# guanjq/targetdiff

Measured on NVIDIA H100. Metric: molecules/sec (1000-step sampling, CrossDocked pocket shape), higher is better.
Workload: dtype f32 (storage, LayerNorm, softmax, accumulation); GEMM operands as 2-piece bf16 splits on wgmma (3 products, ~16-bit operand mantissa)

## Files before the change

### targetdiff_b200/csrc/edge_mlp_v4.cu

```cuda
#include <stdio.h>
#include <stdlib.h>
#include <string.h>

#include "tdiff_common.cuh"
#include "hopper_mma.cuh"

namespace v4 {

constexpr int kCons = 2;
constexpr int kThreads = (kCons + 1) * 128;
constexpr int kTile = 64;
constexpr int kTabClassBytes = 2 * 128 * 128;
constexpr int kProdRegs = 40, kConsRegs = 232;
constexpr int kSrcStride = 512 + 32, kDst = 8;
constexpr int sSrc = 0, sDstRows = sSrc + kTile * kSrcStride, sMeta = sDstRows + kDst * 512, kStage = sMeta + kTile * 16;
constexpr int kMAtom = 32 * 128, kMPiece = 2 * kMAtom, kMImg = 2 * kMPiece;
template <bool FOLD>
struct Map {
  static constexpr int W = 0, T = W + 4 * 128 * 128, Par = T + (FOLD ? 1 : 2) * kTabClassBytes, X = Par + 2 * 128 * 4,
                       M = X + kCons * 4 * 2 * 128 * 4, C = M + (FOLD ? kCons * kMImg : 0), Stage = C + (FOLD ? kCons * 32 * 4 : 0),
                       Bar = Stage + kCons * kStage, Smem = Bar + 8 * (1 + 2 * kCons);
  static_assert(M % 1024 == 0 && Stage % 128 == 0 && kStage % 128 == 0 && Smem <= 227 * 1024, "shared-memory map");
};
constexpr int kOrderBar = 5;
constexpr int kFoldBar = 7;

__device__ __forceinline__ uint32_t smem_u32(const void* p) { return (uint32_t)__cvta_generic_to_shared(p); }
__device__ __forceinline__ void mbar_init(uint32_t bar, uint32_t count) {
  asm volatile("mbarrier.init.shared::cta.b64 [%0], %1;" ::"r"(bar), "r"(count) : "memory");
}
__device__ __forceinline__ void mbar_wait(uint32_t bar, uint32_t parity) {
  asm volatile(
      "{\n\t.reg .pred p;\n\tWAIT_LOOP:\n\tmbarrier.try_wait.parity.shared::cta.b64 p, [%0], %1;\n\t@p bra WAIT_DONE;\n\tbra WAIT_LOOP;\n\t"
      "WAIT_DONE:\n\t}" ::"r"(bar), "r"(parity) : "memory");
}
__device__ __forceinline__ void mbar_expect_tx(uint32_t bar, uint32_t bytes) {
  asm volatile("mbarrier.arrive.expect_tx.shared::cta.b64 _, [%0], %1;" ::"r"(bar), "r"(bytes) : "memory");
}
__device__ __forceinline__ void bulk_g2s(uint32_t smem_dst, const void* gsrc, uint32_t bytes, uint32_t bar) {
  asm volatile("cp.async.bulk.shared::cluster.global.mbarrier::complete_tx::bytes [%0], [%1], %2, [%3];" ::"r"(smem_dst), "l"(gsrc), "r"(bytes),
               "r"(bar) : "memory");
}
__device__ __forceinline__ void fence_barrier_init() { asm volatile("fence.mbarrier_init.release.cluster;" ::: "memory"); }
__device__ __forceinline__ void mbar_arrive(uint32_t bar) { asm volatile("mbarrier.arrive.shared::cta.b64 _, [%0];" ::"r"(bar) : "memory"); }
__device__ __forceinline__ void mbar_expect_tx_only(uint32_t bar, uint32_t bytes) {
  asm volatile("mbarrier.expect_tx.shared::cta.b64 [%0], %1;" ::"r"(bar), "r"(bytes) : "memory");
}
__device__ __forceinline__ void named_bar_sync(int id, int nthreads) { asm volatile("bar.sync %0, %1;" ::"r"(id), "r"(nthreads) : "memory"); }
__device__ __forceinline__ void named_bar_arrive(int id, int nthreads) { asm volatile("bar.arrive %0, %1;" ::"r"(id), "r"(nthreads) : "memory"); }
template <int N> __device__ __forceinline__ void setmaxnreg_inc() { asm volatile("setmaxnreg.inc.sync.aligned.u32 %0;" ::"n"(N)); }
template <int N> __device__ __forceinline__ void setmaxnreg_dec() { asm volatile("setmaxnreg.dec.sync.aligned.u32 %0;" ::"n"(N)); }

__device__ __forceinline__ uint32_t cvt_bf16x2(float hi, float lo) {
  uint32_t d;
  asm("cvt.rn.bf16x2.f32 %0, %1, %2;" : "=r"(d) : "f"(hi), "f"(lo));
  return d;
}
__device__ __forceinline__ float ex2_approx(float x) { float y; asm("ex2.approx.ftz.f32 %0, %1;" : "=f"(y) : "f"(x)); return y; }
__device__ __forceinline__ void stg64(float* p, float a, float b) { asm volatile("st.global.v2.f32 [%0], {%1,%2};" ::"l"(p), "f"(a), "f"(b) : "memory"); }
__device__ __forceinline__ void stg128(float* p, float a, float b, float c, float d) {
  asm volatile("st.global.v4.f32 [%0], {%1,%2,%3,%4};" ::"l"(p), "f"(a), "f"(b), "f"(c), "f"(d) : "memory");
}

struct LnParams { float b[128]; float b2[128]; float mu[20]; };
struct AggArgs {
  const float* logits;
  const float* e_w;
  float* h;
  int key_softmax;
};

template <int N, int M, int LO_BIT>
__device__ __forceinline__ void transpose_reduce(float (&t)[N], int lane) {
  if constexpr (N > M) {
    constexpr int h = (N / M / 2) << LO_BIT;
    const bool up = lane & h;
#pragma unroll
    for (int i = 0; i < N / 2; ++i) {
      const float send = up ? t[i] : t[i + N / 2];
      const float keep = up ? t[i + N / 2] : t[i];
      t[i] = keep + __shfl_xor_sync(0xffffffffu, send, h);
    }
    transpose_reduce<N / 2, M, LO_BIT>(reinterpret_cast<float(&)[N / 2]>(t), lane);
  }
}
__device__ __forceinline__ void split2(float y0, float y1, uint32_t& hi, uint32_t& lo) {
  hi = cvt_bf16x2(y1, y0);
  const float r0 = __fsub_rn(y0, __uint_as_float(hi << 16)), r1 = __fsub_rn(y1, __uint_as_float(hi & 0xffff0000u));
  lo = cvt_bf16x2(r1, r0);
}

}

using namespace v4;

template <int NOUT, bool FOLD>
__global__ void __launch_bounds__(kThreads, 1)
edge_mlp_v4_kernel(const float* __restrict__ P, int zero_row, const int* __restrict__ src, const unsigned char* __restrict__ etype,
                   const float* __restrict__ dist_arr, const int* __restrict__ row_nodes, long long n_dst, long long split_dst,
                   const int* __restrict__ d_counts, int k, int offA, int offB, const unsigned char* __restrict__ w2_image,
                   const unsigned char* __restrict__ tab_image, float coeff, const float* __restrict__ qnode, float* __restrict__ out, int out_by_slot, AggArgs agg,
                   int fold_cls, const __grid_constant__ LnParams lp) {
  static_assert(!FOLD || NOUT == 128, "the fold applies to the key MLPs");
  using L = Map<FOLD>;
  extern __shared__ __align__(1024) unsigned char smem_raw[];
  const uint32_t sbase = smem_u32(smem_raw);
  const uint32_t sW = sbase + L::W, sT = sbase + L::T, sBar = sbase + L::Bar;
  float* const s_b = reinterpret_cast<float*>(smem_raw + L::Par);
  float* const s_b2 = s_b + 128;
  const int tid = threadIdx.x, lane = tid & 31, warp = __shfl_sync(0xffffffffu, tid >> 5, 0);
  const int w = warp & 3, q = lane & 3;
  const int kshift = (k & (k - 1)) == 0 ? __ffs(k) - 1 : -1;
  auto row_dst = [&](long long idx, int& j) -> unsigned {
    const unsigned a = kshift >= 0 ? (unsigned)idx >> kshift : (unsigned)idx / (unsigned)k;
    j = (int)((unsigned)idx - a * (unsigned)k);
    return a;
  };

  if ((sbase & 1023u) != 0) __trap();
  if (d_counts) { n_dst = d_counts[0]; split_dst = d_counts[1]; }
  const long long n_rows = n_dst * k, split_rows = split_dst * k;
  long long row_lo = 0, row_hi = n_rows;
  if constexpr (FOLD) { if (fold_cls) row_lo = split_rows; else row_hi = split_rows; }
  const long long n_tiles = row_hi > row_lo ? (row_hi - row_lo + kTile - 1) / kTile : 0;
  const long long my_tiles = (n_tiles > blockIdx.x) ? (n_tiles - blockIdx.x + gridDim.x - 1) / gridDim.x : 0;
  auto full_bar = [&](int c) { return sBar + 8u * (1 + c); };
  auto empty_bar = [&](int c) { return sBar + 8u * (1 + kCons + c); };

  constexpr int kWAtom = NOUT * 128;
  constexpr int kWPiece = 2 * kWAtom;
  if (tid == 0) {
    mbar_init(sBar, 1);
    for (int c = 0; c < kCons; ++c) { mbar_init(full_bar(c), 32); mbar_init(empty_bar(c), 128); }
    fence_barrier_init();
    if constexpr (FOLD) {
      mbar_expect_tx(sBar, 4u * 128 * 128 + kTabClassBytes);
      bulk_g2s(sW, w2_image, 4u * 128 * 128, sBar);
      bulk_g2s(sT, tab_image + (size_t)fold_cls * kTabClassBytes, kTabClassBytes, sBar);
    } else {
      mbar_expect_tx(sBar, 2u * kWPiece + 2u * kTabClassBytes);
      bulk_g2s(sW, w2_image, 2u * kWPiece, sBar);
      bulk_g2s(sT, tab_image, 2u * kTabClassBytes, sBar);
    }
  }
  for (int i = tid; i < 128; i += kThreads) { s_b[i] = lp.b[i]; s_b2[i] = lp.b2[i]; }
  __syncthreads();

  if (warp < 4) {
    setmaxnreg_dec<kProdRegs>();
    if (warp >= kCons) return;
    const int c = warp;
    const uint32_t st = sbase + L::Stage + (uint32_t)c * kStage;
    for (long long it = c, use = 0; it < my_tiles; it += kCons, ++use) {
      const long long tile = blockIdx.x + it * (long long)gridDim.x, row0 = row_lo + tile * kTile;
      int j0;
      const unsigned a0 = row_dst(row0, j0);
      const long long last = (row0 + kTile - 1 < row_hi ? row0 + kTile - 1 : row_hi - 1);
      const int n_d = min(kDst, (int)(row_dst(last, j0) - a0) + 1);
      int s[2];
      int4 meta[2];
#pragma unroll
      for (int h = 0; h < 2; ++h) {
        const long long idx = row0 + lane + 32 * h;
        int jj = 0, ty = 3, slot = 0, node = -1;
        float dist = 0.f;
        s[h] = -1;
        if (idx < n_rows) {
          const unsigned a = row_dst(idx, jj);
          slot = a - a0 < (unsigned)kDst ? (int)(a - a0) + 1 : 0;
          node = row_nodes[a];
          if (node >= 0) {
            const size_t e = (size_t)node * k + jj;
            s[h] = src[e]; ty = etype[e]; dist = dist_arr[e];
          }
        }
        meta[h] = make_int4(node, s[h], __float_as_int(dist), ty | (slot << 8) | (jj << 16));
      }
      int dnode = -1;
      if (lane < n_d) dnode = row_nodes[a0 + lane];
      mbar_wait(empty_bar(c), (uint32_t)(use & 1) ^ 1u);
#pragma unroll
      for (int h = 0; h < 2; ++h) *reinterpret_cast<int4*>(smem_raw + L::Stage + c * kStage + sMeta + 16 * (lane + 32 * h)) = meta[h];
      if (lane == 0) mbar_expect_tx_only(full_bar(c), (uint32_t)(kTile + (FOLD ? 2 : 1) * n_d) * 512u);
      __syncwarp();
#pragma unroll
      for (int h = 0; h < 2; ++h)
        bulk_g2s(st + sSrc + (uint32_t)(lane + 32 * h) * kSrcStride, P + (size_t)(s[h] >= 0 ? s[h] : zero_row) * TD_NPROJ + offB, 512u, full_bar(c));
      if (lane < n_d) bulk_g2s(st + sDstRows + (uint32_t)lane * 512u, P + (size_t)(dnode >= 0 ? dnode : zero_row) * TD_NPROJ + offA, 512u, full_bar(c));
      if (FOLD && lane < n_d) bulk_g2s(st + sDstRows + (uint32_t)(2 + lane) * 512u, qnode + (size_t)(dnode >= 0 ? dnode : 0) * TD_H, 512u, full_bar(c));
      mbar_arrive(full_bar(c));
    }
    return;
  }

  setmaxnreg_inc<kConsRegs>();
  const int cwg = (warp >> 2) - 1;
  float mu[5];
#pragma unroll
  for (int m = 0; m < 5; ++m) mu[m] = lp.mu[5 * q + m];
  const float coeff2 = coeff * 1.4426950408889634f;
  mbar_wait(sBar, 0);

  const int r_base = 16 * w + (lane >> 2);
  const int pair_bar = 1 + 2 * cwg + (w >> 1);
  float* const xslot = reinterpret_cast<float*>(smem_raw + L::X) + (size_t)(cwg * 4 + w) * 256;
  float* const xpart = xslot + ((w & 1) ? -256 : 256);
  const bool do_agg = !FOLD && NOUT == 128 && qnode == nullptr && agg.logits != nullptr;
  const bool key_sm = NOUT == 128 && qnode != nullptr && agg.key_softmax;
  const unsigned char* const stage = smem_raw + L::Stage + cwg * kStage;
  const int ct = tid & 127, fu = ct & 7, fg = ct >> 3;
  const int fhd = 8 * (fg & 1) + 4 * (fu >> 2) + (fu & 3), fs = fu >> 2, frun = (fg >> 1) ^ (((fu >> 1) & 1) << 2);
  const int fn0 = 16 * ((fhd >> 1) & 1) + 2 * (fhd >> 2) + (fhd & 1);
  unsigned char* const mimg = smem_raw + L::M + cwg * kMImg;
  float* const s_c = reinterpret_cast<float*>(smem_raw + L::C) + cwg * 32;
  const int srow = k == 32 ? (w >> 1) : 0;
  const int order_mine = kOrderBar + cwg, order_other = kOrderBar + (cwg ^ 1);
  const long long n_iter = (my_tiles + kCons - 1) / kCons;
  if (n_iter == 0) return;
  if (cwg == 1) named_bar_arrive(order_other, 256);
  int set = 0;

  for (long long n = 0; n < n_iter; ++n, set ^= 1) {
    const long long it = n * kCons + cwg;
    if (it >= my_tiles) {
      for (int phase = 0; phase < 2; ++phase) { named_bar_sync(order_mine, 256); named_bar_arrive(order_other, 256); }
      continue;
    }
    const long long tile = blockIdx.x + it * (long long)gridDim.x, row0 = row_lo + tile * kTile;
    const int cls = FOLD ? 0 : (row0 >= split_rows) ? 1 : 0;
    long long idx[2];
    int node[2], s[2], ty[2], jj[2], dsl[2];
    float dist[2];
    mbar_wait(full_bar(cwg), (uint32_t)(n & 1));
#pragma unroll
    for (int h = 0; h < 2; ++h) {
      idx[h] = row0 + r_base + 8 * h;
      const int4 m4 = *reinterpret_cast<const int4*>(stage + sMeta + 16 * (r_base + 8 * h));
      node[h] = m4.x; s[h] = m4.y; dist[h] = __int_as_float(m4.z);
      ty[h] = m4.w & 0xff; dsl[h] = ((m4.w >> 8) & 0xff) - 1; jj[h] = m4.w >> 16;
    }
    float ewp[2] = {0.f, 0.f};
    float4 qf[2][2];
    if constexpr (FOLD) {
#pragma unroll
      for (int h = 0; h < 2; ++h)
        if (key_sm && idx[h] < n_rows && node[h] >= 0) ewp[h] = agg.e_w[(size_t)node[h] * k + jj[h]];
#pragma unroll
      for (int sl = 0; sl < 2; ++sl)
#pragma unroll
        for (int hf = 0; hf < 2; ++hf) {
          float4 v = make_float4(0.f, 0.f, 0.f, 0.f);
          if (sl == 0 || k == 32) {
            v = *reinterpret_cast<const float4*>(stage + sDstRows + (2 + sl) * 512 + 32 * fhd + 16 * (hf ^ fs));
            v.x *= 0.35355339059327373f; v.y *= 0.35355339059327373f; v.z *= 0.35355339059327373f; v.w *= 0.35355339059327373f;
          }
          qf[sl][hf] = v;
        }
    }
    uint32_t ghi[4][4], glo[4][4];
#pragma unroll
    for (int h = 0; h < 2; ++h) {
      const bool ok = s[h] >= 0;
      float v[8];
#pragma unroll
      for (int m = 0; m < 5; ++m) {
        const float t = dist[h] - mu[m];
        v[m] = ok ? ex2_approx(coeff2 * (t * t)) : 0.0f;
      }
      v[5] = (ok && q == 3) ? 1.0f : 0.0f;
      v[6] = v[7] = 0.0f;
      const int half = ty[h] < 2 ? 1 : 0;
#pragma unroll
      for (int kk = 0; kk < 4; ++kk)
#pragma unroll
        for (int hk = 0; hk < 2; ++hk) {
          uint32_t hi, lo;
          split2(v[4 * (kk & 1) + 2 * hk], v[4 * (kk & 1) + 2 * hk + 1], hi, lo);
          const bool own = (kk >> 1) == half;
          ghi[kk][h + 2 * hk] = own ? hi : 0u;
          glo[kk][h + 2 * hk] = own ? lo : 0u;
        }
    }
    float x[64];
#pragma unroll
    for (int h = 0; h < 2; ++h) {
      const bool valid = s[h] >= 0;
      const float* ps = reinterpret_cast<const float*>(stage + sSrc + (r_base + 8 * h) * kSrcStride) + 2 * q;
      const float* pd = (dsl[h] >= 0 ? reinterpret_cast<const float*>(stage + sDstRows + dsl[h] * 512)
                                     : P + (size_t)(valid ? node[h] : zero_row) * TD_NPROJ + offA) + 2 * q;
#pragma unroll
      for (int i = 0; i < 16; ++i) {
        const float2 b = *reinterpret_cast<const float2*>(ps + 8 * i);
        float2 a = make_float2(0.f, 0.f);
        if (valid) a = *reinterpret_cast<const float2*>(pd + 8 * i);
        x[4 * i + 2 * h] = __fadd_rn(b.x, a.x);
        x[4 * i + 2 * h + 1] = __fadd_rn(b.y, a.y);
      }
    }
    mbar_arrive(empty_bar(cwg));
    const uint32_t sTc = sT + (uint32_t)cls * kTabClassBytes;
    wgmma_fence();
    named_bar_sync(order_mine, 256);
#pragma unroll
    for (int term = 0; term < 3; ++term) {
#pragma unroll
      for (int kk = 0; kk < 4; ++kk)
        wgmma_n128_rs(x, term == 2 ? glo[kk] : ghi[kk], gmma_desc_sw128(sTc + (term == 1 ? kTabClassBytes / 2 : 0) + kk * 32),
                      1u);
    }
    wgmma_commit();
    named_bar_arrive(order_other, 256);
    if constexpr (FOLD) {
      const float* const w2s = reinterpret_cast<const float*>(smem_raw + L::W) + 8 * fhd;
#pragma unroll
      for (int jr = 0; jr < 2; ++jr) {
        const int f0 = 64 * jr + 8 * frun;
        float mv[2][8];
#pragma unroll
        for (int jf = 0; jf < 8; ++jf) {
          const float4 wa = *reinterpret_cast<const float4*>(w2s + (f0 + jf) * 128 + 4 * fs);
          const float4 wb = *reinterpret_cast<const float4*>(w2s + (f0 + jf) * 128 + 4 * (fs ^ 1));
#pragma unroll
          for (int sl = 0; sl < 2; ++sl) {
            const float4 qa = qf[sl][0], qb = qf[sl][1];
            const float pa = __fmaf_rn(wa.w, qa.w, __fmaf_rn(wa.z, qa.z, __fmaf_rn(wa.y, qa.y, wa.x * qa.x)));
            const float pb = __fmaf_rn(wb.w, qb.w, __fmaf_rn(wb.z, qb.z, __fmaf_rn(wb.y, qb.y, wb.x * qb.x)));
            mv[sl][jf] = pa + pb;
          }
        }
#pragma unroll
        for (int sl = 0; sl < 2; ++sl) {
          uint4 hi, lo;
          split2(mv[sl][0], mv[sl][1], hi.x, lo.x);
          split2(mv[sl][2], mv[sl][3], hi.y, lo.y);
          split2(mv[sl][4], mv[sl][5], hi.z, lo.z);
          split2(mv[sl][6], mv[sl][7], hi.w, lo.w);
          const int nr = fn0 + 8 * sl;
          const int off = jr * kMAtom + (nr >> 3) * 1024 + (nr & 7) * 128 + ((frun ^ (nr & 7)) << 4);
          *reinterpret_cast<uint4*>(mimg + off) = hi;
          *reinterpret_cast<uint4*>(mimg + kMPiece + off) = lo;
        }
      }
      if (fg < 2)
#pragma unroll
        for (int sl = 0; sl < 2; ++sl) {
          const float4 ba = *reinterpret_cast<const float4*>(s_b2 + 8 * fhd + 4 * fs), bb = *reinterpret_cast<const float4*>(s_b2 + 8 * fhd + 4 * (fs ^ 1));
          const float4 qa = qf[sl][0], qb = qf[sl][1];
          const float pa = __fmaf_rn(ba.w, qa.w, __fmaf_rn(ba.z, qa.z, __fmaf_rn(ba.y, qa.y, ba.x * qa.x)));
          const float pb = __fmaf_rn(bb.w, qb.w, __fmaf_rn(bb.z, qb.z, __fmaf_rn(bb.y, qb.y, bb.x * qb.x)));
          s_c[16 * sl + fhd] = pa + pb;
        }
      asm volatile("fence.proxy.async.shared::cta;" ::: "memory");
    }
    wgmma_wait_all();
    float rstd[2];
#pragma unroll
    for (int h = 0; h < 2; ++h) {
      float qa = 0.f, qb = 0.f;
#pragma unroll
      for (int i = 0; i < 16; ++i) {
        qa = __fmaf_rn(x[4 * i + 2 * h], x[4 * i + 2 * h], qa);
        qb = __fmaf_rn(x[4 * i + 2 * h + 1], x[4 * i + 2 * h + 1], qb);
      }
      float var = qa + qb;
      var += __shfl_xor_sync(0xffffffffu, var, 1);
      var += __shfl_xor_sync(0xffffffffu, var, 2);
      rstd[h] = rsqrtf(var * (1.0f / 128.0f) + 1e-5f);
    }
    uint32_t ahi[8][4], alo[8][4];
#pragma unroll
    for (int kk = 0; kk < 8; ++kk)
#pragma unroll
      for (int r = 0; r < 4; ++r) {
        const int h = r & 1, col = 16 * kk + 8 * (r >> 1) + 2 * q, e = 8 * kk + 2 * r;
        const float2 b = *reinterpret_cast<const float2*>(s_b + col);
        const float y0 = __fmaf_rn(x[e], rstd[h], b.x), y1 = __fmaf_rn(x[e + 1], rstd[h], b.y);
        split2(fmaxf(y0, 0.f), fmaxf(y1, 0.f), ahi[kk][r], alo[kk][r]);
      }
    float o[NOUT / 2];
    if constexpr (FOLD) {
      named_bar_sync(kFoldBar + cwg, 128);
#pragma unroll
      for (int sl = 0; sl < 2; ++sl) {
        const float4 cv = *reinterpret_cast<const float4*>(s_c + 16 * sl + 4 * q);
#pragma unroll
        for (int h = 0; h < 2; ++h) {
          o[4 * sl + 2 * h] = cv.x; o[4 * sl + 2 * h + 1] = cv.y;
          o[4 * (2 + sl) + 2 * h] = cv.z; o[4 * (2 + sl) + 2 * h + 1] = cv.w;
        }
      }
    }
    wgmma_fence();
    named_bar_sync(order_mine, 256);
#pragma unroll
    for (int term = 0; term < 3; ++term) {
#pragma unroll
      for (int kk = 0; kk < 8; ++kk) {
        if constexpr (FOLD) {
          const uint64_t desc = gmma_desc_sw128(sbase + L::M + cwg * kMImg + (term == 1 ? kMPiece : 0) + (kk >> 2) * kMAtom + (kk & 3) * 32);
          wgmma_n32_rs(reinterpret_cast<float(&)[16]>(o), term == 2 ? alo[kk] : ahi[kk], desc, 1u);
        } else {
          const uint64_t desc = gmma_desc_sw128(sW + (term == 1 ? kWPiece : 0) + (kk >> 2) * kWAtom + (kk & 3) * 32);
          if constexpr (NOUT == 128) wgmma_n128_rs(o, term == 2 ? alo[kk] : ahi[kk], desc, (term | kk) ? 1u : 0u);
          else wgmma_n16_rs(o, term == 2 ? alo[kk] : ahi[kk], desc, (term | kk) ? 1u : 0u);
        }
      }
    }
    wgmma_commit();
    named_bar_arrive(order_other, 256);
    wgmma_wait_all();

    long long orow[2];
    bool owrite[2];
#pragma unroll
    for (int h = 0; h < 2; ++h) {
      orow[h] = out_by_slot ? ((long long)node[h] * k + jj[h]) : idx[h];
      owrite[h] = idx[h] < n_rows && node[h] >= 0;
    }
    if constexpr (NOUT == 16) {
#pragma unroll
      for (int h = 0; h < 2; ++h)
        if (owrite[h])
#pragma unroll
          for (int i = 0; i < 2; ++i) {
            const float2 bb = *reinterpret_cast<const float2*>(s_b2 + 8 * i + 2 * q);
            stg64(out + (size_t)orow[h] * 16 + 8 * i + 2 * q, o[4 * i + 2 * h] + bb.x, o[4 * i + 2 * h + 1] + bb.y);
          }
    } else if (do_agg) {
      const long long dslot = tile * 2 + (w >> 1);
      const int dnode = dslot < n_dst ? row_nodes[dslot] : -1;
      const bool active = dnode >= 0;
      const int ccol = 64 * (w & 1) + 2 * lane;
      float2 hin = make_float2(0.f, 0.f);
      if (active) hin = *reinterpret_cast<const float2*>(agg.h + (size_t)dnode * TD_H + ccol);
      float wt[2][16];
#pragma unroll
      for (int h = 0; h < 2; ++h)
#pragma unroll
        for (int i = 0; i < 4; ++i) {
          float4 t4 = make_float4(0.f, 0.f, 0.f, 0.f);
          if (active) t4 = __ldg(reinterpret_cast<const float4*>(agg.logits + (size_t)idx[h] * TD_HEADS + 4 * i));
          wt[h][4 * i] = t4.x; wt[h][4 * i + 1] = t4.y; wt[h][4 * i + 2] = t4.z; wt[h][4 * i + 3] = t4.w;
        }
      float t[32];
#pragma unroll
      for (int i = 0; i < 16; ++i) {
        const float2 bb = *reinterpret_cast<const float2*>(s_b2 + 8 * i + 2 * q);
#pragma unroll
        for (int c = 0; c < 2; ++c) {
          const float b = c ? bb.y : bb.x;
          t[2 * i + c] = __fadd_rn(__fmul_rn(__fadd_rn(o[4 * i + c], b), wt[0][i]), __fmul_rn(__fadd_rn(o[4 * i + 2 + c], b), wt[1][i]));
        }
      }
      transpose_reduce<32, 4, 2>(t, lane);
      float* slot = xslot + 128 * set;
      const int c0 = 16 * (lane >> 2) + 2 * q;
      *reinterpret_cast<float2*>(slot + c0) = make_float2(t[0], t[1]);
      *reinterpret_cast<float2*>(slot + c0 + 8) = make_float2(t[2], t[3]);
      named_bar_sync(pair_bar, 64);
      if (active) {
        const float* se = ((w & 1) ? xpart : xslot) + 128 * set;
        const float* so = ((w & 1) ? xslot : xpart) + 128 * set;
        const float2 a = *reinterpret_cast<const float2*>(se + ccol), b = *reinterpret_cast<const float2*>(so + ccol);
        *reinterpret_cast<float2*>(agg.h + (size_t)dnode * TD_H + ccol) = make_float2(hin.x + (a.x + b.x), hin.y + (a.y + b.y));
      }
    } else if (!FOLD && qnode == nullptr) {
#pragma unroll
      for (int h = 0; h < 2; ++h)
        if (owrite[h])
#pragma unroll
          for (int i = 0; i < 16; ++i) {
            const float2 bb = *reinterpret_cast<const float2*>(s_b2 + 8 * i + 2 * q);
            stg64(out + (size_t)orow[h] * 128 + 8 * i + 2 * q, o[4 * i + 2 * h] + bb.x, o[4 * i + 2 * h + 1] + bb.y);
          }
    } else {
      float lg[32];
      if constexpr (FOLD) {
#pragma unroll
        for (int h = 0; h < 2; ++h)
#pragma unroll
          for (int u = 0; u < 4; ++u) {
            const int e0 = 4 * (2 * (u >> 1)) + 2 * h + (u & 1);
            lg[4 * h + u] = srow ? o[e0 + 4] : o[e0];
          }
      } else {
#pragma unroll
        for (int h = 0; h < 2; ++h) {
          const float* qrow = qnode + (size_t)(node[h] >= 0 ? node[h] : 0) * TD_H + 2 * q;
#pragma unroll
          for (int i = 0; i < 16; ++i) {
            const float2 qv = __ldg(reinterpret_cast<const float2*>(qrow + 8 * i));
            const float2 bb = *reinterpret_cast<const float2*>(s_b2 + 8 * i + 2 * q);
            lg[8 * (i >> 2) + 4 * h + (i & 3)] = __fmaf_rn(o[4 * i + 2 * h + 1] + bb.y, qv.y, (o[4 * i + 2 * h] + bb.x) * qv.x);
          }
        }
        transpose_reduce<32, 8, 0>(lg, lane);
#pragma unroll
        for (int u = 0; u < 8; ++u) lg[u] *= 0.35355339059327373f;
      }
      if (key_sm) {
        bool valid_e[2];
        float ew[2];
#pragma unroll
        for (int h = 0; h < 2; ++h) {
          valid_e[h] = false; ew[h] = 0.f;
          if (owrite[h]) {
            valid_e[h] = s[h] >= 0;
            ew[h] = FOLD ? ewp[h] : agg.e_w[(size_t)node[h] * k + jj[h]];
          }
        }
        float mx[4], sm[4];
#pragma unroll
        for (int u = 0; u < 4; ++u) {
          lg[u] = valid_e[0] ? lg[u] * 1.4426950408889634f : -INFINITY;
          lg[4 + u] = valid_e[1] ? lg[4 + u] * 1.4426950408889634f : -INFINITY;
          mx[u] = fmaxf(lg[u], lg[4 + u]);
#pragma unroll
          for (int m = 4; m < 32; m <<= 1) mx[u] = fmaxf(mx[u], __shfl_xor_sync(0xffffffffu, mx[u], m));
        }
        if (lane < 4) *reinterpret_cast<float4*>(xslot + 4 * q) = make_float4(mx[0], mx[1], mx[2], mx[3]);
        named_bar_sync(pair_bar, 64);
        const float4 pm = *reinterpret_cast<const float4*>(xpart + 4 * q);
        mx[0] = fmaxf(mx[0], pm.x); mx[1] = fmaxf(mx[1], pm.y); mx[2] = fmaxf(mx[2], pm.z); mx[3] = fmaxf(mx[3], pm.w);
#pragma unroll
        for (int u = 0; u < 4; ++u) {
          lg[u] = valid_e[0] ? ex2_approx(lg[u] - mx[u]) : 0.0f;
          lg[4 + u] = valid_e[1] ? ex2_approx(lg[4 + u] - mx[u]) : 0.0f;
          sm[u] = lg[u] + lg[4 + u];
#pragma unroll
          for (int m = 4; m < 32; m <<= 1) sm[u] += __shfl_xor_sync(0xffffffffu, sm[u], m);
        }
        if (lane < 4) *reinterpret_cast<float4*>(xslot + 128 + 4 * q) = make_float4(sm[0], sm[1], sm[2], sm[3]);
        named_bar_sync(pair_bar, 64);
        const float4 ps = *reinterpret_cast<const float4*>(xpart + 128 + 4 * q);
        const float pl[4] = {ps.x, ps.y, ps.z, ps.w};
#pragma unroll
        for (int u = 0; u < 4; ++u) {
          const float l = sm[u] + pl[u];
          const float inv = l > 0.0f ? 1.0f / l : 0.0f;
          lg[u] = lg[u] * ew[0] * inv;
          lg[4 + u] = lg[4 + u] * ew[1] * inv;
        }
#pragma unroll
        for (int h = 0; h < 2; ++h)
          if (idx[h] < n_rows) stg128(out + (size_t)idx[h] * TD_HEADS + 4 * q, lg[4 * h], lg[4 * h + 1], lg[4 * h + 2], lg[4 * h + 3]);
      } else {
#pragma unroll
        for (int h = 0; h < 2; ++h)
          if (owrite[h]) stg128(out + (size_t)orow[h] * TD_HEADS + 4 * q, lg[4 * h], lg[4 * h + 1], lg[4 * h + 2], lg[4 * h + 3]);
      }
    }
  }
  if (cwg == 0) named_bar_sync(order_mine, 256);
}

void td_launch_edge_mlp_v4(const float* P, int zero_row, const int* src, const unsigned char* etype, const float* dist, const int* row_nodes, long long n_dst,
                           long long split_dst, const int* d_counts, int k, const TdMlp& m, const float* h_offsets, float coeff,
                           const float* h_ln_b, const float* h_b2, const float* qnode, float* out, int out_by_slot,
                           const float* agg_logits, const float* agg_e_w, float* agg_h, int key_softmax, int sm_count, cudaStream_t st) {
  if (n_dst == 0) return;
  LnParams lp;
  memcpy(lp.b, h_ln_b, sizeof(lp.b));
  memset(lp.b2, 0, sizeof(lp.b2));
  memcpy(lp.b2, h_b2, sizeof(float) * (size_t)m.nout);
  memcpy(lp.mu, h_offsets, sizeof(lp.mu));
  static size_t opted128[TD_MAX_DEVICES] = {0}, opted16[TD_MAX_DEVICES] = {0}, optedF[TD_MAX_DEVICES] = {0};
  td_opt_in_smem(edge_mlp_v4_kernel<128, false>, Map<false>::Smem, opted128);
  td_opt_in_smem(edge_mlp_v4_kernel<16, false>, Map<false>::Smem, opted16);
  td_opt_in_smem(edge_mlp_v4_kernel<128, true>, Map<true>::Smem, optedF);
  auto grid_of = [&](long long n_dst_range) {
    const long long n_tiles = (n_dst_range * k + kTile - 1) / kTile;
    return (int)(n_tiles < sm_count ? n_tiles : sm_count);
  };
  AggArgs agg = {agg_logits, agg_e_w, agg_h, (key_softmax && k == 32) ? 1 : 0};
  if (m.nout == 16) {
    edge_mlp_v4_kernel<16, false><<<grid_of(n_dst), kThreads, Map<false>::Smem, st>>>(
        P, zero_row, src, etype, dist, row_nodes, n_dst, split_dst, d_counts, k, m.offA, m.offB, m.w2_img, m.tabcls_img, coeff, nullptr, out,
        out_by_slot, agg, 0, lp);
  } else if (qnode && (k == 32 || k == 64)) {
    const long long n_cls[2] = {split_dst, n_dst - split_dst};
    for (int cls = 0; cls < 2; ++cls)
      if (n_cls[cls] > 0)
        edge_mlp_v4_kernel<128, true><<<grid_of(n_cls[cls]), kThreads, Map<true>::Smem, st>>>(
            P, zero_row, src, etype, dist, row_nodes, n_dst, split_dst, d_counts, k, m.offA, m.offB,
            reinterpret_cast<const unsigned char*>(m.w2t), m.tabcls_img, coeff, qnode, out, out_by_slot, agg, cls, lp);
  } else {
    edge_mlp_v4_kernel<128, false><<<grid_of(n_dst), kThreads, Map<false>::Smem, st>>>(
        P, zero_row, src, etype, dist, row_nodes, n_dst, split_dst, d_counts, k, m.offA, m.offB, m.w2_img, m.tabcls_img, coeff, qnode, out,
        out_by_slot, agg, 0, lp);
  }
}
```

### targetdiff_b200/csrc/engine.cu

```cuda
#include <math.h>
#include <stdarg.h>
#include <stdio.h>
#include <stdlib.h>
#include <string.h>

#include <list>
#include <map>
#include <string>
#include <vector>

#include "../../include/tdiff.h"
#include "sampler.cuh"
#include "tdiff_common.cuh"

static thread_local char g_err[1024] = "";
static int set_err(int code, const char* fmt, ...) {
  va_list ap;
  va_start(ap, fmt);
  vsnprintf(g_err, sizeof(g_err), fmt, ap);
  va_end(ap);
  return code;
}
#define CK(call)                                                                                       \
  do {                                                                                                 \
    cudaError_t _e = (call);                                                                           \
    if (_e != cudaSuccess) return set_err(TDIFF_ECUDA, "%s failed: %s (%s:%d)", #call, cudaGetErrorString(_e), __FILE__, __LINE__); \
  } while (0)

struct DevBuf {
  void* p = nullptr;
  size_t cap = 0;
  int ensure(size_t bytes) {
    if (bytes <= cap) return 0;
    if (p) cudaFree(p);
    p = nullptr; cap = 0;
    size_t want = bytes + bytes / 8 + 256;
    if (cudaMalloc(&p, want) != cudaSuccess) { (void)cudaGetLastError(); if (cudaMalloc(&p, bytes) != cudaSuccess) { (void)cudaGetLastError(); return -1; } want = bytes; }
    cap = want;
    static const bool poison = getenv("TDIFF_POISON") != nullptr;
    if (poison) cudaMemset(p, 0xFF, want);
    return 0;
  }
  void release() { if (p) cudaFree(p); p = nullptr; cap = 0; }
  template <class T> T* as() const { return reinterpret_cast<T*>(p); }
};

struct TdLayer {
  std::vector<TdSubLayer> x2h, h2x;
  const float* offsets;
  float coeff;
};

enum { EV_AGG_H = 0, EV_AGG_X = 1, EV_EDGE_MLP = 2, EV_TOTAL = 3, EV_KINDS = 4 };
struct EvPair { cudaEvent_t a, b; int kind; };

struct tdiff_engine {
  tdiff_config cfg;
  int device = 0, sm_count = 132;
  float* arena = nullptr;
  std::vector<float> host_arena;
  unsigned char* img_arena = nullptr;
  int mlp_mode = 2;
  bool mlp_v4 = true;
  std::vector<TdLayer> layers;
  const float *w_prot = nullptr, *b_prot = nullptr, *wl_t = nullptr, *bl = nullptr;
  const float *ew_w1t = nullptr, *ew_b1 = nullptr, *ew_g = nullptr, *ew_b = nullptr, *ew_w2 = nullptr, *ew_off = nullptr;
  float ew_b2 = 0.f, ew_coeff = -0.5f;
  int num_blocks = 1, ew_mode = 0 , out_fc = 0, time_emb = 0;
  int num_x2h = 1, num_h2x = 1, sync_twoup = 0;
  const float* w_time = nullptr;
  const float* zeros128 = nullptr;
  DevBuf ew_x2h, ew_h2x, hagg, time_norm;
  DevBuf h_sync;
  const float *hd_w1t = nullptr, *hd_b1 = nullptr, *hd_w2 = nullptr, *hd_b2 = nullptr;
  const float *t_c0 = nullptr, *t_ct = nullptr, *t_logvar = nullptr, *t_la = nullptr, *t_l1ma = nullptr, *t_lca = nullptr, *t_l1mca = nullptr,
              *t_sra = nullptr, *t_srm1 = nullptr;
  bool bound = false, has_ligand = false, have_graph = false;
  bool restrict_last = false;
  bool knn_incremental = false;
  bool have_prev = false;
  bool env_no_fused_agg = false, env_no_restrict = false, env_no_graph = false, env_knn_full = false, env_no_slot_keep = false;
  int B = 0, N = 0, Np = 0, Nl = 0, K = 0, max_ng = 0, final_buf = 0;
  int KQ = 0, hybrid = 0;
  DevBuf node_ptr, prot_ptr, prot_node, prot_graph, lig_node, lig_graph, node_lig;
  DevBuf rel_flag, rel_list, n_rel, work_list, n_work, knn_cache;
  DevBuf x2h_rows, lig_rows, rel_rows, rel_counts;
  long long x2h_n_dst = 0, x2h_split = 0, lig_n_dst = 0;
  int row_pad = 4;
  int free_depth = 0;
  int env_free_depth = 2;
  bool free_ready = false;
  DevBuf h_free, dirty, free_rows, free_counts, lig_save;
  long long free_stride = 0;
  DevBuf xm0, xm1, offset, h0, h, P, q, src, src_prev, etype, e_w, dist, kbuf, vbuf, v16, lig_pos, lig_v, logits;
  DevBuf step, err_flag, node_off, total_edges;
  DevBuf stage[8];
  cudaStream_t own_stream = nullptr;
  cudaEvent_t ev_fork = nullptr, ev_join = nullptr;
  long long launches = 0;
  bool profiling = false;
  std::vector<EvPair> events;
  double ms_acc[EV_KINDS] = {0, 0, 0, 0};
  long long n_acc[EV_KINDS] = {0, 0, 0, 0};
};

namespace {
struct Packer {
  std::map<std::string, const tdiff_tensor*> byname;
  std::vector<float> host;
  std::vector<unsigned char> img;
  std::string missing;
  std::list<std::vector<float>> keep;
  const float* get(const std::string& name, int64_t numel) {
    auto it = byname.find(name);
    if (it == byname.end() || it->second->numel != numel || it->second->data == nullptr) {
      if (missing.empty()) missing = name + (it == byname.end() ? " (absent)" : " (wrong size)");
      return nullptr;
    }
    return it->second->data;
  }
  size_t alloc(size_t n) {
    size_t off = (host.size() + 63) / 64 * 64;
    host.resize(off + n, 0.0f);
    return off;
  }
};

struct MlpOff { size_t tab, ln_g, ln_b, w2t, b2; int nout; long long img, tabcls; };

inline uint16_t bf16_rn(float x) {
  uint32_t u; memcpy(&u, &x, 4);
  if ((u & 0x7fffffffu) > 0x7f800000u) return (uint16_t)((u >> 16) | 0x40);
  u += 0x7fffu + ((u >> 16) & 1u);
  return (uint16_t)(u >> 16);
}
inline float bf16_f(uint16_t b) { uint32_t u = (uint32_t)b << 16; float f; memcpy(&f, &u, 4); return f; }

void pack_umma_image(const float* w2, std::vector<unsigned char>& img, size_t off, int nrows = 128) {
  for (int n = 0; n < nrows; ++n)
    for (int kk = 0; kk < 128; ++kk) {
      float r = w2[(size_t)n * 128 + kk];
      const size_t o = (size_t)(kk / 64) * ((size_t)nrows * 128) + (size_t)n * 128 + (size_t)((((kk % 64) / 8) ^ (n & 7)) * 16) + (size_t)(kk % 8) * 2;
      for (int p = 0; p < 3; ++p) {
        const uint16_t b = bf16_rn(r);
        r = r - bf16_f(b);
        memcpy(&img[off + (size_t)p * ((size_t)nrows * 256) + o], &b, 2);
      }
    }
}

void pack_tabcls_image(const float* tab , std::vector<unsigned char>& img, size_t off) {
  static const int type_of[2][2] = {{3, 1}, {2, 0}};
  for (int cls = 0; cls < 2; ++cls)
    for (int n = 0; n < 128; ++n)
      for (int slot = 0; slot < 64; ++slot) {
        const int half = slot >> 5, sl = slot & 31;
        const int q = (sl & 7) >> 1, m = 2 * (sl >> 3) + (sl & 1);
        int j = -1;
        if (m < 5) j = 5 * q + m;
        else if (m == 5 && q == 3) j = 20;
        float r = j >= 0 ? tab[((size_t)type_of[cls][half] * TD_TAB + j) * TD_H + n] : 0.0f;
        const size_t o = (size_t)n * 128 + (size_t)(((slot >> 3) ^ (n & 7)) * 16) + (size_t)(slot & 7) * 2;
        for (int p = 0; p < 2; ++p) {
          const uint16_t b = bf16_rn(r);
          r = r - bf16_f(b);
          memcpy(&img[off + (size_t)cls * 32768 + (size_t)p * 16384 + o], &b, 2);
        }
      }
}

bool pack_edge_mlp(Packer& pk, const std::string& p, int nout, bool sign_in_w1, MlpOff& o, const float** w1_out) {
  const int KV = 4 + 4 * TD_NG + 2 * TD_H;
  const float* w1_in = pk.get(p + ".net.0.weight", (int64_t)TD_H * KV);
  const float* b1_in = pk.get(p + ".net.0.bias", TD_H);
  const float* g_in = pk.get(p + ".net.1.weight", TD_H);
  const float* b_in = pk.get(p + ".net.1.bias", TD_H);
  const float* w2_in = pk.get(p + ".net.3.weight", (int64_t)nout * TD_H);
  const float* b2_in = pk.get(p + ".net.3.bias", nout);
  if (!w1_in || !b1_in || !g_in || !b_in || !w2_in || !b2_in) return false;
  std::vector<float>& w1v = pk.keep.emplace_back((size_t)TD_H * KV);
  std::vector<float> b1v(TD_H), gv(TD_H), bv(TD_H), w2v((size_t)nout * TD_H), b2v(nout);
  {
    std::vector<double> mw(KV, 0.0), b2acc(b2_in, b2_in + nout);
    double mb = 0.0;
    for (int f = 0; f < TD_H; ++f) {
      for (int j = 0; j < KV; ++j) mw[j] += w1_in[(size_t)f * KV + j];
      mb += b1_in[f];
    }
    for (int f = 0; f < TD_H; ++f) {
      const double s = g_in[f] < 0.0f ? -1.0 : 1.0, ag = fabs((double)g_in[f]), s1 = sign_in_w1 ? s : 1.0;
      for (int j = 0; j < KV; ++j) w1v[(size_t)f * KV + j] = (float)(s1 * (w1_in[(size_t)f * KV + j] - mw[j] / TD_H));
      b1v[f] = (float)(s1 * (b1_in[f] - mb / TD_H));
      gv[f] = (float)(s / s1);
      const float bf = (float)(b_in[f] / ag);
      const bool constant = g_in[f] == 0.0f || !isfinite(bf);
      bv[f] = constant ? 0.0f : bf;
      for (int n = 0; n < nout; ++n) {
        const double w = w2_in[(size_t)n * TD_H + f];
        w2v[(size_t)n * TD_H + f] = constant ? 0.0f : (float)(ag * w);
        if (constant && b_in[f] > 0.0f) b2acc[n] += (double)b_in[f] * w;
      }
    }
    for (int n = 0; n < nout; ++n) b2v[n] = (float)b2acc[n];
  }
  const float *w1 = w1v.data(), *b1 = b1v.data(), *g = gv.data(), *b = bv.data(), *w2 = w2v.data(), *b2 = b2v.data();
  o.nout = nout;
  o.tab = pk.alloc(4 * TD_TAB * TD_H);
  for (int t = 0; t < 4; ++t) {
    for (int j = 0; j < TD_NG; ++j)
      for (int f = 0; f < TD_H; ++f) pk.host[o.tab + (t * TD_TAB + j) * TD_H + f] = w1[(size_t)f * KV + 4 + t * TD_NG + j];
    for (int f = 0; f < TD_H; ++f) pk.host[o.tab + (t * TD_TAB + TD_NG) * TD_H + f] = w1[(size_t)f * KV + t] + b1[f];
  }
  o.ln_g = pk.alloc(TD_H); memcpy(&pk.host[o.ln_g], g, TD_H * sizeof(float));
  o.ln_b = pk.alloc(TD_H); memcpy(&pk.host[o.ln_b], b, TD_H * sizeof(float));
  o.w2t = pk.alloc((size_t)TD_H * nout);
  for (int kk = 0; kk < TD_H; ++kk)
    for (int n = 0; n < nout; ++n) pk.host[o.w2t + (size_t)kk * nout + n] = w2[(size_t)n * TD_H + kk];
  o.b2 = pk.alloc(nout); memcpy(&pk.host[o.b2], b2, nout * sizeof(float));
  o.img = -1; o.tabcls = -1;
  if (nout == TD_H || nout == 16) {
    o.img = (long long)pk.img.size();
    pk.img.resize(pk.img.size() + 3 * (size_t)nout * 256, 0);
    pack_umma_image(w2, pk.img, (size_t)o.img, nout);
    o.tabcls = (long long)pk.img.size();
    pk.img.resize(pk.img.size() + 2 * 32768, 0);
    pack_tabcls_image(&pk.host[o.tab], pk.img, (size_t)o.tabcls);
  }
  *w1_out = w1;
  return true;
}

struct SubOff {
  size_t wn_t, bn; long long wn_img; MlpOff k, v, q;
  long long ew_w = -1; float ew_b = 0.f;
  long long out_wa = -1, out_wb = -1, out_w2 = -1, out_b1 = -1, out_g = -1, out_b = -1, out_b2 = -1;
};

bool pack_sublayer_options(Packer& pk, const std::string& p, int ew_dim, bool out_fc, SubOff& so) {
  if (ew_dim > 0) {
    const float* w = pk.get(p + ".ew_net.0.weight", ew_dim);
    const float* b = pk.get(p + ".ew_net.0.bias", 1);
    if (!w || !b) return false;
    so.ew_w = (long long)pk.alloc(ew_dim);
    memcpy(&pk.host[so.ew_w], w, ew_dim * sizeof(float));
    so.ew_b = b[0];
  }
  if (out_fc) {
    const std::string np = p + ".node_output";
    const float* w1 = pk.get(np + ".net.0.weight", (int64_t)TD_H * 2 * TD_H);
    const float* b1 = pk.get(np + ".net.0.bias", TD_H);
    const float* g = pk.get(np + ".net.1.weight", TD_H);
    const float* b = pk.get(np + ".net.1.bias", TD_H);
    const float* w2 = pk.get(np + ".net.3.weight", (int64_t)TD_H * TD_H);
    const float* b2 = pk.get(np + ".net.3.bias", TD_H);
    if (!w1 || !b1 || !g || !b || !w2 || !b2) return false;
    std::vector<float> blk((size_t)TD_H * TD_H);
    for (int half = 0; half < 2; ++half) {
      for (int n = 0; n < TD_H; ++n)
        for (int kk = 0; kk < TD_H; ++kk) blk[(size_t)n * TD_H + kk] = w1[(size_t)n * 2 * TD_H + half * TD_H + kk];
      long long& dst = half == 0 ? so.out_wa : so.out_wb;
      dst = (long long)pk.img.size();
      pk.img.resize(pk.img.size() + 3 * 32768, 0);
      pack_umma_image(blk.data(), pk.img, (size_t)dst);
    }
    so.out_w2 = (long long)pk.img.size();
    pk.img.resize(pk.img.size() + 3 * 32768, 0);
    pack_umma_image(w2, pk.img, (size_t)so.out_w2);
    so.out_b1 = (long long)pk.alloc(TD_H); memcpy(&pk.host[so.out_b1], b1, TD_H * 4);
    so.out_g = (long long)pk.alloc(TD_H); memcpy(&pk.host[so.out_g], g, TD_H * 4);
    so.out_b = (long long)pk.alloc(TD_H); memcpy(&pk.host[so.out_b], b, TD_H * 4);
    so.out_b2 = (long long)pk.alloc(TD_H); memcpy(&pk.host[so.out_b2], b2, TD_H * 4);
  }
  return true;
}

bool pack_sublayer(Packer& pk, const std::string& p, const char* kn, const char* vn, const char* qn, int nout_v, bool sign_in_w1, SubOff& so) {
  const int KV = 4 + 4 * TD_NG + 2 * TD_H;
  const float *w1k = nullptr, *w1v = nullptr;
  if (!pack_edge_mlp(pk, p + "." + kn, TD_H, sign_in_w1, so.k, &w1k)) return false;
  if (!pack_edge_mlp(pk, p + "." + vn, nout_v, sign_in_w1, so.v, &w1v)) return false;
  const std::string qp = p + "." + qn;
  const float* w1q = pk.get(qp + ".net.0.weight", (int64_t)TD_H * TD_H);
  const float* b1q = pk.get(qp + ".net.0.bias", TD_H);
  const float* gq = pk.get(qp + ".net.1.weight", TD_H);
  const float* bq = pk.get(qp + ".net.1.bias", TD_H);
  const float* w2q = pk.get(qp + ".net.3.weight", (int64_t)TD_H * TD_H);
  const float* b2q = pk.get(qp + ".net.3.bias", TD_H);
  if (!w1q || !b1q || !gq || !bq || !w2q || !b2q) return false;
  so.q.nout = TD_H; so.q.tab = 0; so.q.tabcls = -1;
  so.q.img = (long long)pk.img.size();
  pk.img.resize(pk.img.size() + 3 * 32768, 0);
  pack_umma_image(w2q, pk.img, (size_t)so.q.img);
  so.q.ln_g = pk.alloc(TD_H); memcpy(&pk.host[so.q.ln_g], gq, TD_H * sizeof(float));
  so.q.ln_b = pk.alloc(TD_H); memcpy(&pk.host[so.q.ln_b], bq, TD_H * sizeof(float));
  so.q.w2t = pk.alloc((size_t)TD_H * TD_H);
  for (int kk = 0; kk < TD_H; ++kk)
    for (int n = 0; n < TD_H; ++n) pk.host[so.q.w2t + (size_t)kk * TD_H + n] = w2q[(size_t)n * TD_H + kk];
  so.q.b2 = pk.alloc(TD_H); memcpy(&pk.host[so.q.b2], b2q, TD_H * sizeof(float));
  so.wn_t = pk.alloc((size_t)TD_H * TD_NPROJ);
  so.bn = pk.alloc(TD_NPROJ);
  for (int kk = 0; kk < TD_H; ++kk) {
    float* row = &pk.host[so.wn_t + (size_t)kk * TD_NPROJ];
    for (int c = 0; c < TD_H; ++c) {
      row[c] = w1k[(size_t)c * KV + 4 + 4 * TD_NG + kk];
      row[128 + c] = w1v[(size_t)c * KV + 4 + 4 * TD_NG + kk];
      row[256 + c] = w1k[(size_t)c * KV + 4 + 4 * TD_NG + TD_H + kk];
      row[384 + c] = w1v[(size_t)c * KV + 4 + 4 * TD_NG + TD_H + kk];
      row[512 + c] = w1q[(size_t)c * TD_H + kk];
    }
  }
  for (int c = 0; c < TD_H; ++c) pk.host[so.bn + 512 + c] = b1q[c];
  so.wn_img = (long long)pk.img.size();
  pk.img.resize(pk.img.size() + 5 * 3 * 32768, 0);
  std::vector<float> blk((size_t)TD_H * TD_H);
  for (int y = 0; y < 5; ++y) {
    for (int n = 0; n < TD_H; ++n)
      for (int kk = 0; kk < TD_H; ++kk) blk[(size_t)n * TD_H + kk] = pk.host[so.wn_t + (size_t)kk * TD_NPROJ + y * TD_H + n];
    pack_umma_image(blk.data(), pk.img, (size_t)so.wn_img + (size_t)y * 3 * 32768);
  }
  return true;
}

TdMlp mk_mlp(const float* base, const unsigned char* img_base, const MlpOff& o, int offA, int offB) {
  TdMlp m;
  m.w2_img = (o.img >= 0 && img_base) ? img_base + o.img : nullptr;
  m.tabcls_img = (o.tabcls >= 0 && img_base) ? img_base + o.tabcls : nullptr;
  m.tab = base + o.tab; m.ln_g = base + o.ln_g; m.ln_b = base + o.ln_b; m.w2t = base + o.w2t; m.b2 = base + o.b2;
  m.nout = o.nout; m.offA = offA; m.offB = offB;
  return m;
}
}

extern "C" const char* tdiff_last_error(void) { return g_err; }
extern "C" const char* tdiff_version(void) { return "tdiff-b200 0.1 (sm_90a)"; }

extern "C" int tdiff_create(const tdiff_config* cfg, const tdiff_tensor* sd, int n_entries, int device, tdiff_engine** out) {
  if (!cfg || !sd || !out) return set_err(TDIFF_EINVAL, "null argument");
  *out = nullptr;
  if (cfg->hidden_dim != TD_H || cfg->n_heads != TD_HEADS || cfg->num_r_gaussian != TD_NG)
    return set_err(TDIFF_EINVAL, "unsupported model shape: hidden_dim=%d n_heads=%d num_r_gaussian=%d (kernels are built for 128/16/20)",
                   cfg->hidden_dim, cfg->n_heads, cfg->num_r_gaussian);
  if (cfg->knn < 1 || cfg->knn > TD_KMAX) return set_err(TDIFF_EINVAL, "knn=%d outside 1..%d", cfg->knn, TD_KMAX);
  if (cfg->model_mean_type != 0 && cfg->model_mean_type != 1)
    return set_err(TDIFF_EINVAL, "model_mean_type=%d (0 = C0, 1 = noise)", cfg->model_mean_type);
  for (int r : cfg->reserved)
    if (r != 0) return set_err(TDIFF_EINVAL, "tdiff_config.reserved must be 0");
  int num_x2h = 1, num_h2x = 1, sync_twoup = 0;
  if (cfg->sublayers != 0) {
    const unsigned s = (unsigned)cfg->sublayers;
    num_x2h = (int)(s & 0xffu); num_h2x = (int)((s >> 8) & 0xffu); sync_twoup = (int)((s >> 16) & 0xffu);
    if ((s >> 24) != 1u || num_x2h > 16 || num_h2x > 16 || sync_twoup > 1)
      return set_err(TDIFF_EINVAL, "sublayers=0x%08x: expected 0 or 1<<24 | sync_twoup<<16 | num_h2x<<8 | num_x2h with num_x2h, num_h2x in 0..16 and "
                     "sync_twoup in 0..1", s);
  }
  if (cfg->cutoff_mode != 0 && cfg->cutoff_mode != 1) return set_err(TDIFF_EINVAL, "cutoff_mode=%d (0 = 'knn', 1 = 'hybrid')", cfg->cutoff_mode);
  if (cfg->num_blocks < 0 || cfg->num_blocks > 16 || cfg->ew_net_type < 0 || cfg->ew_net_type > 3 || (cfg->x2h_out_fc != 0 && cfg->x2h_out_fc != 1) ||
      (cfg->time_emb != 0 && cfg->time_emb != 1))
    return set_err(TDIFF_EINVAL, "bad option (num_blocks=%d ew_net_type=%d x2h_out_fc=%d time_emb=%d)", cfg->num_blocks, cfg->ew_net_type,
                   cfg->x2h_out_fc, cfg->time_emb);
  if (cfg->num_layers < 1 || cfg->num_classes < 1 || cfg->num_classes > TD_CMAX || cfg->protein_feat_dim < 1 || cfg->num_timesteps < 1)
    return set_err(TDIFF_EINVAL, "bad config (num_layers=%d num_classes=%d protein_feat_dim=%d num_timesteps=%d)", cfg->num_layers,
                   cfg->num_classes, cfg->protein_feat_dim, cfg->num_timesteps);
  int ndev = 0;
  if (cudaGetDeviceCount(&ndev) != cudaSuccess || ndev == 0) {
    (void)cudaGetLastError();
    return set_err(TDIFF_ECUDA, "no CUDA device: libtdiff has no CPU fallback");
  }
  if (device < 0 || device >= ndev) return set_err(TDIFF_EINVAL, "device %d out of range (%d devices)", device, ndev);
  CK(cudaSetDevice(device));
  cudaDeviceProp prop;
  CK(cudaGetDeviceProperties(&prop, device));
  if (prop.major != 9) return set_err(TDIFF_ECUDA, "device %d is sm_%d%d; this library is built for sm_90a only", device, prop.major, prop.minor);

  tdiff_engine* e = new tdiff_engine();
  e->cfg = *cfg; e->device = device; e->sm_count = prop.multiProcessorCount; e->K = e->KQ = cfg->knn; e->hybrid = cfg->cutoff_mode;
  e->num_blocks = cfg->num_blocks > 1 ? cfg->num_blocks : 1; e->ew_mode = cfg->ew_net_type; e->out_fc = cfg->x2h_out_fc; e->time_emb = cfg->time_emb;
  e->num_x2h = num_x2h; e->num_h2x = num_h2x; e->sync_twoup = sync_twoup;
  if (const char* mode = getenv("TDIFF_EDGE_MLP")) {
    if (!strcmp(mode, "simt")) e->mlp_mode = 0;
    else if (!strcmp(mode, "tc3")) e->mlp_mode = 2;
    else if (!strcmp(mode, "tc3v2")) { e->mlp_mode = 2; e->mlp_v4 = false; }
    else if (!strcmp(mode, "tc6")) e->mlp_mode = 3;
    else { delete e; return set_err(TDIFF_EINVAL, "TDIFF_EDGE_MLP=%s (simt|tc3|tc3v2|tc6)", mode); }
  }
  const bool v4 = e->mlp_mode == 2 && e->mlp_v4;

  Packer pk;
  for (int i = 0; i < n_entries; ++i)
    if (sd[i].name) pk.byname[sd[i].name] = &sd[i];
  const int T = cfg->num_timesteps, KC = cfg->num_classes, F = cfg->protein_feat_dim, L = cfg->num_layers;
  struct { const char* name; size_t off; } tabs[9] = {{"posterior_mean_c0_coef", 0}, {"posterior_mean_ct_coef", 0}, {"posterior_logvar", 0},
      {"log_alphas_v", 0}, {"log_one_minus_alphas_v", 0}, {"log_alphas_cumprod_v", 0}, {"log_one_minus_alphas_cumprod_v", 0},
      {"sqrt_recip_alphas_cumprod", 0}, {"sqrt_recipm1_alphas_cumprod", 0}};
  for (auto& t : tabs) {
    const float* p = pk.get(t.name, T);
    t.off = pk.alloc(T);
    if (p) memcpy(&pk.host[t.off], p, T * sizeof(float));
  }
  const float* wp = pk.get("protein_atom_emb.weight", (int64_t)(TD_H - 1) * F);
  const float* bp = pk.get("protein_atom_emb.bias", TD_H - 1);
  const int KIN = KC + (cfg->time_emb ? 1 : 0);
  const float* wl = pk.get("ligand_atom_emb.weight", (int64_t)(TD_H - 1) * KIN);
  const float* blp = pk.get("ligand_atom_emb.bias", TD_H - 1);
  size_t o_wp = pk.alloc((size_t)TD_H * F), o_bp = pk.alloc(TD_H), o_wl = pk.alloc((size_t)KC * TD_H), o_bl = pk.alloc(TD_H),
         o_wtime = pk.alloc(TD_H), o_zeros = pk.alloc(TD_H);
  if (wp && bp && wl && blp) {
    memcpy(&pk.host[o_wp], wp, (size_t)(TD_H - 1) * F * sizeof(float));
    memcpy(&pk.host[o_bp], bp, (TD_H - 1) * sizeof(float));
    for (int v = 0; v < KC; ++v)
      for (int f = 0; f < TD_H - 1; ++f) pk.host[o_wl + (size_t)v * TD_H + f] = wl[(size_t)f * KIN + v];
    if (cfg->time_emb)
      for (int f = 0; f < TD_H - 1; ++f) pk.host[o_wtime + f] = wl[(size_t)f * KIN + KC];
    memcpy(&pk.host[o_bl], blp, (TD_H - 1) * sizeof(float));
  }
  const bool has_gate = cfg->ew_net_type == 0;
  const float* gw1 = has_gate ? pk.get("refine_net.edge_pred_layer.net.0.weight", (int64_t)TD_H * TD_NG) : nullptr;
  const float* gb1 = has_gate ? pk.get("refine_net.edge_pred_layer.net.0.bias", TD_H) : nullptr;
  const float* gg = has_gate ? pk.get("refine_net.edge_pred_layer.net.1.weight", TD_H) : nullptr;
  const float* gb = has_gate ? pk.get("refine_net.edge_pred_layer.net.1.bias", TD_H) : nullptr;
  const float* gw2 = has_gate ? pk.get("refine_net.edge_pred_layer.net.3.weight", TD_H) : nullptr;
  const float* gb2 = has_gate ? pk.get("refine_net.edge_pred_layer.net.3.bias", 1) : nullptr;
  const float* goff = pk.get("refine_net.distance_expansion.offset", TD_NG);
  size_t o_gw1 = pk.alloc((size_t)TD_NG * TD_H), o_gb1 = pk.alloc(TD_H), o_gg = pk.alloc(TD_H), o_gb = pk.alloc(TD_H), o_gw2 = pk.alloc(TD_H),
         o_goff = pk.alloc(TD_NG);
  if (goff) memcpy(&pk.host[o_goff], goff, TD_NG * 4);
  if (gw1 && gb1 && gg && gb && gw2 && gb2 && goff) {
    for (int j = 0; j < TD_NG; ++j)
      for (int f = 0; f < TD_H; ++f) pk.host[o_gw1 + (size_t)j * TD_H + f] = gw1[(size_t)f * TD_NG + j];
    memcpy(&pk.host[o_gb1], gb1, TD_H * 4); memcpy(&pk.host[o_gg], gg, TD_H * 4); memcpy(&pk.host[o_gb], gb, TD_H * 4);
    memcpy(&pk.host[o_gw2], gw2, TD_H * 4); memcpy(&pk.host[o_goff], goff, TD_NG * 4);
    e->ew_b2 = gb2[0];
    const float d = goff[1] - goff[0];
    e->ew_coeff = -0.5f / (d * d);
  }
  const float* hw1 = pk.get("v_inference.0.weight", (int64_t)TD_H * TD_H);
  const float* hb1 = pk.get("v_inference.0.bias", TD_H);
  const float* hw2 = pk.get("v_inference.2.weight", (int64_t)KC * TD_H);
  const float* hb2 = pk.get("v_inference.2.bias", KC);
  size_t o_hw1 = pk.alloc((size_t)TD_H * TD_H), o_hb1 = pk.alloc(TD_H), o_hw2 = pk.alloc((size_t)KC * TD_H), o_hb2 = pk.alloc(KC);
  if (hw1 && hb1 && hw2 && hb2) {
    for (int kk = 0; kk < TD_H; ++kk)
      for (int n = 0; n < TD_H; ++n) pk.host[o_hw1 + (size_t)kk * TD_H + n] = hw1[(size_t)n * TD_H + kk];
    memcpy(&pk.host[o_hb1], hb1, TD_H * 4); memcpy(&pk.host[o_hw2], hw2, (size_t)KC * TD_H * 4); memcpy(&pk.host[o_hb2], hb2, KC * 4);
  }
  std::vector<std::vector<SubOff>> sx(L, std::vector<SubOff>(num_x2h)), sh(L, std::vector<SubOff>(num_h2x));
  std::vector<size_t> o_off(L);
  std::vector<float> coeffs(L, -0.5f);
  for (int l = 0; l < L; ++l) {
    const std::string p = "refine_net.base_block." + std::to_string(l);
    bool ok = true;
    for (int i = 0; ok && i < num_x2h; ++i) ok = pack_sublayer(pk, p + ".x2h_layers." + std::to_string(i), "hk_func", "hv_func", "hq_func", TD_H, v4, sx[l][i]);
    for (int i = 0; ok && i < num_h2x; ++i) ok = pack_sublayer(pk, p + ".h2x_layers." + std::to_string(i), "xk_func", "xv_func", "xq_func", TD_HEADS, v4, sh[l][i]);
    for (int i = 0; ok && i < num_x2h; ++i)
      ok = pack_sublayer_options(pk, p + ".x2h_layers." + std::to_string(i), cfg->ew_net_type == 1 ? 4 * TD_NG : cfg->ew_net_type == 2 ? TD_H : 0,
                                 cfg->x2h_out_fc != 0, sx[l][i]);
    for (int i = 0; ok && i < num_h2x; ++i)
      ok = pack_sublayer_options(pk, p + ".h2x_layers." + std::to_string(i), cfg->ew_net_type == 1 ? 4 * TD_NG : 0, false, sh[l][i]);
    if (!ok) break;
    const float* off = pk.get(p + ".distance_expansion.offset", TD_NG);
    o_off[l] = pk.alloc(TD_NG);
    if (off) {
      memcpy(&pk.host[o_off[l]], off, TD_NG * 4);
      const float d = off[1] - off[0];
      coeffs[l] = -0.5f / (d * d);
    }
  }
  if (!pk.missing.empty()) {
    delete e;
    return set_err(TDIFF_EWEIGHT, "state_dict entry %s", pk.missing.c_str());
  }
  const size_t bytes = pk.host.size() * sizeof(float);
  if (cudaMalloc(&e->arena, bytes) != cudaSuccess) { delete e; return set_err(TDIFF_ECUDA, "cudaMalloc(%zu) for weights failed", bytes); }
  if (cudaMemcpy(e->arena, pk.host.data(), bytes, cudaMemcpyHostToDevice) != cudaSuccess) {
    cudaFree(e->arena); delete e; return set_err(TDIFF_ECUDA, "weight upload failed");
  }
  if (!pk.img.empty()) {
    if (cudaMalloc(&e->img_arena, pk.img.size()) != cudaSuccess ||
        cudaMemcpy(e->img_arena, pk.img.data(), pk.img.size(), cudaMemcpyHostToDevice) != cudaSuccess) {
      cudaFree(e->arena); delete e; return set_err(TDIFF_ECUDA, "weight image upload failed");
    }
  }
  if ((cfg->ew_net_type != 0 || cfg->x2h_out_fc || cfg->cutoff_mode != 0) && !(e->mlp_mode == 2 && e->mlp_v4)) {
    cudaFree(e->arena); cudaFree(e->img_arena); delete e;
    return set_err(TDIFF_EINVAL, "ew_net_type != 'global', x2h_out_fc and cutoff_mode 'hybrid' are implemented (and tested) in the default engine mode only (unset TDIFF_EDGE_MLP)");
  }
  if (cfg->sublayers != 0 && !(num_x2h == 1 && num_h2x == 1 && !sync_twoup) && !(e->mlp_mode == 2 && e->mlp_v4)) {
    cudaFree(e->arena); cudaFree(e->img_arena); delete e;
    return set_err(TDIFF_EINVAL, "num_x2h / num_h2x != 1 and sync_twoup are implemented (and tested) in the default engine mode only (unset TDIFF_EDGE_MLP)");
  }
  e->env_no_fused_agg = getenv("TDIFF_NO_FUSED_AGG") != nullptr;
  e->env_no_restrict = getenv("TDIFF_NO_RESTRICT") != nullptr;
  e->env_no_graph = getenv("TDIFF_NO_GRAPH") != nullptr;
  e->env_knn_full = getenv("TDIFF_KNN_FULL") != nullptr;
  e->env_no_slot_keep = getenv("TDIFF_NO_SLOT_KEEP") != nullptr;
  if (const char* fd = getenv("TDIFF_FREE_DEPTH")) e->env_free_depth = atoi(fd) < 0 ? 0 : (atoi(fd) > 8 ? 8 : atoi(fd));
  e->host_arena = pk.host;
  const float* A = e->arena;
  const unsigned char* IM = e->img_arena;
  e->t_c0 = A + tabs[0].off; e->t_ct = A + tabs[1].off; e->t_logvar = A + tabs[2].off; e->t_la = A + tabs[3].off;
  e->t_l1ma = A + tabs[4].off; e->t_lca = A + tabs[5].off; e->t_l1mca = A + tabs[6].off;
  e->t_sra = A + tabs[7].off; e->t_srm1 = A + tabs[8].off;
  e->w_prot = A + o_wp; e->b_prot = A + o_bp; e->wl_t = A + o_wl; e->bl = A + o_bl;
  e->w_time = cfg->time_emb ? A + o_wtime : nullptr; e->zeros128 = A + o_zeros;
  e->ew_w1t = A + o_gw1; e->ew_b1 = A + o_gb1; e->ew_g = A + o_gg; e->ew_b = A + o_gb; e->ew_w2 = A + o_gw2; e->ew_off = A + o_goff;
  e->hd_w1t = A + o_hw1; e->hd_b1 = A + o_hb1; e->hd_w2 = A + o_hw2; e->hd_b2 = A + o_hb2;
  e->layers.resize(L);
  for (int l = 0; l < L; ++l) {
    TdLayer& ly = e->layers[l];
    ly.offsets = A + o_off[l]; ly.coeff = coeffs[l];
    ly.x2h.resize(num_x2h); ly.h2x.resize(num_h2x);
    for (int idx = 0; idx < num_x2h + num_h2x; ++idx) {
      const bool is_h2x = idx >= num_x2h;
      TdSubLayer& sl = is_h2x ? ly.h2x[idx - num_x2h] : ly.x2h[idx];
      const SubOff& so = is_h2x ? sh[l][idx - num_x2h] : sx[l][idx];
      sl.wn_t = A + so.wn_t; sl.bn = A + so.bn; sl.wn_img = IM ? IM + so.wn_img : nullptr;
      sl.k = mk_mlp(A, IM, so.k, 0, 256); sl.v = mk_mlp(A, IM, so.v, 128, 384); sl.q = mk_mlp(A, IM, so.q, 512, 512);
      sl.ew_w = so.ew_w >= 0 ? A + so.ew_w : nullptr; sl.ew_b = so.ew_b;
      sl.out_wa_img = so.out_wa >= 0 ? IM + so.out_wa : nullptr; sl.out_wb_img = so.out_wb >= 0 ? IM + so.out_wb : nullptr;
      sl.out_b1 = so.out_b1 >= 0 ? A + so.out_b1 : nullptr;
      memset(&sl.out, 0, sizeof(sl.out));
      if (so.out_w2 >= 0) {
        sl.out.w2_img = IM + so.out_w2; sl.out.ln_g = A + so.out_g; sl.out.ln_b = A + so.out_b; sl.out.b2 = A + so.out_b2; sl.out.nout = TD_H;
      }
    }
  }
  if (e->step.ensure(sizeof(int)) || e->err_flag.ensure(sizeof(int)) || e->total_edges.ensure(sizeof(long long))) {
    tdiff_destroy(e); return set_err(TDIFF_ECUDA, "cudaMalloc failed");
  }
  cudaMemset(e->err_flag.p, 0, sizeof(int));
  if (cudaStreamCreateWithFlags(&e->own_stream, cudaStreamNonBlocking) != cudaSuccess ||
      cudaEventCreateWithFlags(&e->ev_fork, cudaEventDisableTiming) != cudaSuccess ||
      cudaEventCreateWithFlags(&e->ev_join, cudaEventDisableTiming) != cudaSuccess) {
    tdiff_destroy(e); return set_err(TDIFF_ECUDA, "stream/event creation failed");
  }
  *out = e;
  return TDIFF_OK;
}

extern "C" void tdiff_destroy(tdiff_engine* e) {
  if (!e) return;
  cudaSetDevice(e->device);
  for (auto& ev : e->events) { cudaEventDestroy(ev.a); cudaEventDestroy(ev.b); }
  if (e->own_stream) cudaStreamDestroy(e->own_stream);
  if (e->ev_fork) cudaEventDestroy(e->ev_fork);
  if (e->ev_join) cudaEventDestroy(e->ev_join);
  DevBuf* bufs[] = {&e->node_ptr, &e->prot_ptr, &e->prot_node, &e->prot_graph, &e->lig_node, &e->lig_graph, &e->node_lig, &e->xm0, &e->xm1,
                    &e->rel_flag, &e->rel_list, &e->n_rel, &e->work_list, &e->n_work, &e->knn_cache, &e->x2h_rows, &e->lig_rows, &e->rel_rows, &e->rel_counts, &e->ew_x2h, &e->ew_h2x, &e->h_sync, &e->hagg, &e->time_norm, &e->h_free, &e->dirty, &e->free_rows, &e->free_counts, &e->lig_save, &e->offset, &e->h0, &e->h, &e->P, &e->q, &e->src, &e->src_prev, &e->etype, &e->e_w, &e->dist, &e->kbuf, &e->vbuf, &e->v16, &e->lig_pos,
                    &e->lig_v, &e->logits, &e->step, &e->err_flag, &e->node_off, &e->total_edges};
  for (auto* b : bufs) b->release();
  for (auto& b : e->stage) b.release();
  if (e->arena) cudaFree(e->arena);
  if (e->img_arena) cudaFree(e->img_arena);
  delete e;
}

extern "C" int tdiff_bind_batch(tdiff_engine* e, int B, const int32_t* pc, const int32_t* lc, const float* d_ppos, const float* d_pfeat,
                                int center_mode, void* stream) {
  if (!e || !pc || !lc || B < 1) return set_err(TDIFF_EINVAL, "bind_batch: bad arguments");
  if (center_mode != 0 && center_mode != 1) return set_err(TDIFF_EINVAL, "center_mode %d (0 'none' | 1 'protein')", center_mode);
  cudaStream_t st = (cudaStream_t)stream;
  CK(cudaSetDevice(e->device));
  long long N = 0, Np = 0, Nl = 0;
  int max_ng = 0;
  for (int g = 0; g < B; ++g) {
    if (pc[g] < 0 || lc[g] < 0) return set_err(TDIFF_EINVAL, "negative atom count in graph %d", g);
    Np += pc[g]; Nl += lc[g];
    if (pc[g] + lc[g] > max_ng) max_ng = pc[g] + lc[g];
  }
  N = Np + Nl;
  if (N <= 0) return set_err(TDIFF_EINVAL, "empty batch");
  if (e->hybrid) {
    int max_lc = 0;
    for (int g = 0; g < B; ++g) {
      if (lc[g] > max_lc) max_lc = lc[g];
      if (lc[g] > 0 && pc[g] < e->KQ)
        return set_err(TDIFF_EINVAL, "cutoff_mode 'hybrid': graph %d has %d protein atoms < k = %d (torch.topk fails in the reference too)", g, pc[g], e->KQ);
    }
    const int need = e->KQ + (max_lc > 0 ? max_lc - 1 : 0);
    if (need > TD_KMAX)
      return set_err(TDIFF_EINVAL, "cutoff_mode 'hybrid': k + n_ligand - 1 = %d + %d - 1 exceeds the %d neighbour slots per node", e->KQ, max_lc, TD_KMAX);
    e->K = need;
  }
  if (N * (long long)e->K >= (1LL << 31) / 1) return set_err(TDIFF_EINVAL, "batch too large: N*k = %lld edge slots", N * e->K);
  if (max_ng > 2800) return set_err(TDIFF_EINVAL, "graph with %d nodes exceeds the k-NN kernel's shared-memory tile (2800)", max_ng);
  if (Np > 0 && (!d_ppos || !d_pfeat)) return set_err(TDIFF_EINVAL, "null protein arrays");
  const int K = e->K;
  std::vector<int> node_ptr(B + 1), prot_ptr(B + 1), prot_node(Np), prot_graph(Np), lig_node(Nl), lig_graph(Nl), node_lig(N, -1);
  int n = 0, p = 0, a = 0;
  for (int g = 0; g < B; ++g) {
    node_ptr[g] = n; prot_ptr[g] = p;
    for (int i = 0; i < pc[g]; ++i) { prot_node[p] = n; prot_graph[p] = g; ++p; ++n; }
    for (int i = 0; i < lc[g]; ++i) { lig_node[a] = n; lig_graph[a] = g; node_lig[n] = a; ++a; ++n; }
  }
  node_ptr[B] = n; prot_ptr[B] = p;
  e->bound = false; e->has_ligand = false; e->have_graph = false; e->have_prev = false;
  e->B = B; e->N = (int)N; e->Np = (int)Np; e->Nl = (int)Nl; e->max_ng = max_ng;
  const size_t slots = (size_t)N * K;
  int bad = 0;
  bad |= e->node_ptr.ensure((B + 1) * 4) | e->prot_ptr.ensure((B + 1) * 4) | e->prot_node.ensure(Np * 4 + 4) | e->prot_graph.ensure(Np * 4 + 4);
  bad |= e->lig_node.ensure(Nl * 4 + 4) | e->lig_graph.ensure(Nl * 4 + 4) | e->node_lig.ensure(N * 4);
  bad |= e->xm0.ensure(N * 16) | e->xm1.ensure(N * 16) | e->offset.ensure((size_t)B * 16);
  bad |= e->h0.ensure(N * TD_H * 4) | e->h.ensure(N * TD_H * 4) | e->P.ensure((size_t)(N + 1) * TD_NPROJ * 4) | e->q.ensure(N * TD_H * 4);
  bad |= e->src.ensure(slots * 4) | e->src_prev.ensure(slots * 4) | e->etype.ensure(slots) | e->e_w.ensure(slots * 4) | e->dist.ensure(slots * 4);
  const bool v4 = e->mlp_mode == 2 && e->mlp_v4;
  int gcd128 = 128;
  while (K % gcd128) gcd128 >>= 1;
  e->row_pad = 128 / gcd128;
  const long long pad = e->row_pad, nPpad = (Np + pad - 1) / pad * pad, nLpad = (Nl + pad - 1) / pad * pad;
  e->x2h_n_dst = nPpad + nLpad; e->x2h_split = nPpad; e->lig_n_dst = nLpad;
  std::vector<int> x2h_rows((size_t)(nPpad + nLpad), -1), lig_rows((size_t)nLpad, -1);
  for (long long i = 0; i < Np; ++i) x2h_rows[i] = prot_node[i];
  for (long long i = 0; i < Nl; ++i) { x2h_rows[nPpad + i] = lig_node[i]; lig_rows[i] = lig_node[i]; }
  if (v4) bad |= e->x2h_rows.ensure(x2h_rows.size() * 4 + 4) | e->lig_rows.ensure(lig_rows.size() * 4 + 4) | e->rel_rows.ensure(x2h_rows.size() * 4 + 4) |
                 e->rel_counts.ensure(16);
  const bool fuse = v4 && K == 32 && !e->env_no_fused_agg && e->ew_mode != 2;
  if (e->ew_mode == 1) bad |= e->ew_x2h.ensure(slots * 4) | e->ew_h2x.ensure(slots * 4);
  if (e->out_fc) bad |= e->hagg.ensure((size_t)N * TD_H * 4);
  if (e->sync_twoup && e->num_x2h > 0 && e->num_h2x > 0) bad |= e->h_sync.ensure((size_t)N * TD_H * 4);
  if (e->time_emb) bad |= e->time_norm.ensure((size_t)B * 4 + 16);
  bad |= e->kbuf.ensure(v4 ? (size_t)(nPpad + nLpad) * K * TD_HEADS * 4 + 64 : slots * TD_H * 4);
  if (!fuse) bad |= e->vbuf.ensure(slots * TD_H * 4);
  bad |= e->v16.ensure((size_t)nLpad * K * TD_HEADS * 4 + 16);
  int min_pc = 1 << 30;
  for (int g = 0; g < B; ++g) if (pc[g] < min_pc) min_pc = pc[g];
  e->free_ready = false;
  e->free_depth = (fuse && !e->hybrid && Nl > 0 && min_pc > K) ? e->env_free_depth : 0;
  const int x2h_evals = (int)e->layers.size() * e->num_x2h;
  if (e->free_depth > x2h_evals - 1) e->free_depth = x2h_evals - 1 > 0 ? x2h_evals - 1 : 0;
  if (e->free_depth > 0)
    bad |= e->h_free.ensure((size_t)e->free_depth * N * TD_H * 4) | e->dirty.ensure((size_t)e->free_depth * N + 16) |
           e->free_rows.ensure((size_t)e->free_depth * x2h_rows.size() * 4 + 4) | e->free_counts.ensure((size_t)e->free_depth * 16) |
           e->lig_save.ensure((size_t)Nl * 20 + 32);
  e->free_stride = (long long)x2h_rows.size();
  bad |= e->lig_pos.ensure(Nl * 16 + 16) | e->lig_v.ensure(Nl * 4 + 4) | e->logits.ensure((size_t)Nl * e->cfg.num_classes * 4 + 4);
  bad |= e->node_off.ensure(N * 8) | e->rel_flag.ensure(N + 16) | e->rel_list.ensure(N * 4 + 64) | e->n_rel.ensure(16) | e->work_list.ensure(N * 4 + 64) | e->n_work.ensure(16);
  e->knn_incremental = !e->env_knn_full && Np > 0;
  if (e->knn_incremental) bad |= e->knn_cache.ensure((size_t)N * (e->KQ + 1) * 8);
  if (bad) return set_err(TDIFF_ECUDA, "out of device memory binding a batch of %lld nodes (%zu edge slots)", N, slots);
  CK(cudaMemcpyAsync(e->node_ptr.p, node_ptr.data(), (B + 1) * 4, cudaMemcpyHostToDevice, st));
  CK(cudaMemcpyAsync(e->prot_ptr.p, prot_ptr.data(), (B + 1) * 4, cudaMemcpyHostToDevice, st));
  if (Np) {
    CK(cudaMemcpyAsync(e->prot_node.p, prot_node.data(), Np * 4, cudaMemcpyHostToDevice, st));
    CK(cudaMemcpyAsync(e->prot_graph.p, prot_graph.data(), Np * 4, cudaMemcpyHostToDevice, st));
  }
  if (Nl) {
    CK(cudaMemcpyAsync(e->lig_node.p, lig_node.data(), Nl * 4, cudaMemcpyHostToDevice, st));
    CK(cudaMemcpyAsync(e->lig_graph.p, lig_graph.data(), Nl * 4, cudaMemcpyHostToDevice, st));
  }
  CK(cudaMemcpyAsync(e->node_lig.p, node_lig.data(), N * 4, cudaMemcpyHostToDevice, st));
  if (v4) {
    if (!x2h_rows.empty()) CK(cudaMemcpyAsync(e->x2h_rows.p, x2h_rows.data(), x2h_rows.size() * 4, cudaMemcpyHostToDevice, st));
    if (!lig_rows.empty()) CK(cudaMemcpyAsync(e->lig_rows.p, lig_rows.data(), lig_rows.size() * 4, cudaMemcpyHostToDevice, st));
  }
  CK(cudaStreamSynchronize(st));
  CK(cudaMemsetAsync(e->offset.p, 0, (size_t)B * 16, st));
  if (e->time_emb) CK(cudaMemsetAsync(e->time_norm.p, 0, (size_t)B * 4, st));
  CK(cudaMemsetAsync(e->h0.p, 0, (size_t)N * TD_H * 4, st));
  CK(cudaMemsetAsync(e->xm0.p, 0, (size_t)N * 16, st));
  CK(cudaMemsetAsync(e->xm1.p, 0, (size_t)N * 16, st));
  CK(cudaMemsetAsync(e->etype.p, 0, slots, st));
  CK(cudaMemsetAsync(e->P.as<float>() + (size_t)N * TD_NPROJ, 0, (size_t)TD_NPROJ * 4, st));
  if (center_mode == 1) td_launch_segment_mean3(d_ppos, e->prot_ptr.as<int>(), B, e->offset.as<float4>(), st);
  td_launch_place_protein(d_ppos, e->prot_node.as<int>(), e->prot_graph.as<int>(), e->offset.as<float4>(), (int)Np, e->xm0.as<float4>(),
                          e->xm1.as<float4>(), st);
  td_launch_protein_embed(d_pfeat, (int)Np, e->cfg.protein_feat_dim, e->w_prot, e->b_prot, e->prot_node.as<int>(), e->h0.as<float>(), st);
  e->launches += 3;
  if (e->knn_incremental) {
    td_launch_knn_cache(e->xm0.as<float4>(), e->node_ptr.as<int>(), e->prot_ptr.as<int>(), B, max_ng, e->KQ, e->knn_cache.as<unsigned long long>(), st);
    e->launches += 1;
  }
  CK(cudaGetLastError());
  e->bound = true;
  return TDIFF_OK;
}

extern "C" int tdiff_set_ligand(tdiff_engine* e, const float* d_pos, const int64_t* d_v, int apply_center, void* stream) {
  if (!e || !e->bound) return set_err(TDIFF_ESTATE, "set_ligand before bind_batch");
  if (e->Nl > 0 && !d_pos) return set_err(TDIFF_EINVAL, "null ligand positions");
  if (!e->has_ligand && e->Nl > 0 && !d_v) return set_err(TDIFF_EINVAL, "ligand types required on first set_ligand");
  cudaStream_t st = (cudaStream_t)stream;
  CK(cudaSetDevice(e->device));
  td_launch_set_ligand(d_pos, (const long long*)d_v, e->lig_graph.as<int>(), e->offset.as<float4>(), apply_center, e->Nl,
                       e->cfg.num_classes, e->lig_pos.as<float4>(), e->lig_v.as<int>(), e->err_flag.as<int>(), st);
  e->launches += 1;
  if (d_v) {
    int flag = 0;
    CK(cudaMemcpyAsync(&flag, e->err_flag.p, sizeof(int), cudaMemcpyDeviceToHost, st));
    CK(cudaStreamSynchronize(st));
    if (flag) {
      cudaMemsetAsync(e->err_flag.p, 0, sizeof(int), st);
      e->has_ligand = false;
      return set_err(TDIFF_EINVAL, "ligand atom type index >= num_classes (%d)", e->cfg.num_classes);
    }
  }
  CK(cudaGetLastError());
  e->has_ligand = true;
  return TDIFF_OK;
}

extern "C" int tdiff_get_ligand(tdiff_engine* e, float* d_pos, int64_t* d_v, int add_offset, void* stream) {
  if (!e || !e->has_ligand) return set_err(TDIFF_ESTATE, "get_ligand before set_ligand");
  CK(cudaSetDevice(e->device));
  td_launch_get_ligand(e->lig_pos.as<float4>(), e->lig_v.as<int>(), e->lig_graph.as<int>(), e->offset.as<float4>(), add_offset, e->Nl, d_pos,
                       (long long*)d_v, (cudaStream_t)stream);
  e->launches += 1;
  CK(cudaGetLastError());
  return TDIFF_OK;
}

extern "C" int tdiff_get_offset(tdiff_engine* e, float* d_offset, void* stream) {
  if (!e || !e->bound || !d_offset) return set_err(TDIFF_ESTATE, "get_offset before bind_batch");
  CK(cudaSetDevice(e->device));
  td_launch_gather_xyz(e->offset.as<float4>(), nullptr, e->B, d_offset, (cudaStream_t)stream);
  e->launches += 1;
  CK(cudaGetLastError());
  return TDIFF_OK;
}

namespace {
struct Prof {
  tdiff_engine* e; cudaStream_t st; int kind; bool on; EvPair ev;
  Prof(tdiff_engine* e_, cudaStream_t st_, int kind_) : e(e_), st(st_), kind(kind_), on(e_->profiling) {
    if (on) { cudaEventCreate(&ev.a); cudaEventCreate(&ev.b); ev.kind = kind; cudaEventRecord(ev.a, st); }
  }
  ~Prof() { if (on) { cudaEventRecord(ev.b, st); e->events.push_back(ev); } }
};

enum RowList { ROWS_ALL = 0, ROWS_LIGAND = 1, ROWS_RELEVANT = 2 };
bool fused_logits(const tdiff_engine* e) { return e->mlp_mode == 2 && e->mlp_v4; }
void edge_mlp(tdiff_engine* e, const float* P, const float4* xm, const int* src, const unsigned char* etype, RowList list, int K, const TdMlp& m,
              const float* offsets, float coeff, float* out, cudaStream_t st, const float* e_w, const float* qnode = nullptr,
              const float* agg_logits = nullptr, float* agg_h = nullptr, int key_softmax = 0, int free_layer = -1) {
  if (fused_logits(e) && m.w2_img && m.tabcls_img) {
    const int* rows = list == ROWS_ALL ? e->x2h_rows.as<int>() : list == ROWS_LIGAND ? e->lig_rows.as<int>() : e->rel_rows.as<int>();
    const int* counts = list == ROWS_RELEVANT ? e->rel_counts.as<int>() : nullptr;
    if (free_layer >= 0) {
      rows = e->free_rows.as<int>() + (size_t)free_layer * e->free_stride;
      counts = e->free_counts.as<int>() + 4 * free_layer;
    }
    const long long n_dst = list == ROWS_LIGAND ? e->lig_n_dst : e->x2h_n_dst;
    const long long split = list == ROWS_LIGAND ? 0 : e->x2h_split;
    const int by_slot = (list != ROWS_LIGAND && !key_softmax && agg_logits == nullptr) ? 1 : 0;
    td_launch_edge_mlp_v4(P, e->N, src, etype, e->dist.as<float>(), rows, n_dst, split, counts, K, m,
                          e->host_arena.data() + (offsets - e->arena), coeff, e->host_arena.data() + (m.ln_b - e->arena),
                          e->host_arena.data() + (m.b2 - e->arena), qnode, out, by_slot, agg_logits, e_w, agg_h, key_softmax,
                          e->sm_count, st);
    return;
  }
  const int* row_nodes = list == ROWS_LIGAND ? e->lig_node.as<int>() : nullptr;
  const long long n_rows = (long long)(list == ROWS_LIGAND ? e->Nl : e->N) * K;
  if (e->mlp_mode != 0 && m.nout == TD_H && m.w2_img)
    td_launch_edge_mlp_tc(P, xm, src, etype, e->dist.as<float>(), row_nodes, n_rows, K, m, m.w2_img, e->mlp_mode, offsets, coeff, out, e->sm_count, st);
  else
    td_launch_edge_mlp(P, xm, src, etype, row_nodes, n_rows, K, m, offsets, coeff, out, e->sm_count, st);
}

void node_side(tdiff_engine* e, const float* h, int N, const TdSubLayer& sl, float* P, float* q, cudaStream_t st, const int* rows = nullptr,
               const int* d_n = nullptr) {
  if (e->mlp_mode != 0 && sl.wn_img && sl.q.w2_img) {
    TdMlp pm = sl.q;
    pm.b2 = sl.bn;
    td_launch_rows_tc(1, h, TD_H, 0, N, pm, sl.wn_img, e->mlp_mode, P, TD_NPROJ, TD_NPROJ / TD_H, rows, d_n, e->sm_count, st);
    td_launch_rows_tc(2, P, TD_NPROJ, 512, N, sl.q, sl.q.w2_img, e->mlp_mode, q, TD_H, 1, rows, d_n, e->sm_count, st);
  } else {
    td_launch_node_proj(h, N, sl.wn_t, sl.bn, P, st);
    td_launch_node_q(P, N, sl.q, q, st);
  }
}

void run_forward(tdiff_engine* e, cudaStream_t st, int fix_x, int free_build = 0, float* blk_pos = nullptr, float* blk_logits = nullptr) {
  const int N = e->N, Nl = e->Nl, K = e->K;
  float4* xm[2] = {e->xm0.as<float4>(), e->xm1.as<float4>()};
  const int* src = e->src.as<int>();
  const unsigned char* etype = e->etype.as<unsigned char>();
  float* h = e->h.as<float>();
  float* P = e->P.as<float>();
  float* q = e->q.as<float>();
  td_launch_scatter_ligand_pos(e->lig_pos.as<float4>(), e->lig_node.as<int>(), Nl, xm[0], st);
  td_launch_init_h(e->h0.as<float>(), xm[0], e->lig_v.as<int>(), e->node_lig.as<int>(), e->wl_t, e->bl, e->w_time, e->time_norm.as<float>(),
                   e->lig_graph.as<int>(), N, h, st);
  e->launches += 2;
  int cur = 0;
  const int KC = e->cfg.num_classes;
  auto snapshot = [&](int i) {
    if (blk_pos) {
      td_launch_gather_xyz(xm[cur], e->lig_node.as<int>(), Nl, blk_pos + (size_t)i * Nl * 3, st);
      e->launches += 1;
    }
    if (blk_logits) {
      td_launch_head(h, e->lig_node.as<int>(), Nl, e->hd_w1t, e->hd_b1, e->hd_w2, e->hd_b2, KC, blk_logits + (size_t)i * Nl * KC, st);
      e->launches += 1;
    }
  };
  if (Nl > 0) snapshot(0);
  const int n_blocks = free_build ? 1 : e->num_blocks;
  for (int blk = 0; blk < n_blocks; ++blk) {
    const int use_free = (!free_build && e->free_ready && blk == 0) ? e->free_depth : 0;
    const bool last_blk = blk + 1 == n_blocks;
    if (e->knn_incremental)
      td_launch_knn_update(xm[cur], e->node_ptr.as<int>(), e->prot_ptr.as<int>(), e->B, e->max_ng, e->KQ, K, e->hybrid, e->knn_cache.as<unsigned long long>(),
                           e->src.as<int>(), st);
    else
      td_launch_knn(xm[cur], e->node_ptr.as<int>(), e->prot_ptr.as<int>(), e->B, e->max_ng, e->KQ, K, e->hybrid, e->src.as<int>(), st);
    td_launch_edge_const(xm[cur], src, e->src_prev.as<int>(), e->have_prev ? 1 : 0, N, K, e->ew_off, e->ew_coeff, e->ew_w1t, e->ew_b1, e->ew_g, e->ew_b, e->ew_w2,
                         e->ew_b2, e->etype.as<unsigned char>(), e->e_w.as<float>(), e->rel_flag.as<unsigned char>(),
                         use_free ? e->dirty.as<unsigned char>() : nullptr, e->work_list.as<int>(), e->n_work.as<int>(), (e->ew_mode != 0 ? 1 : 0) | (e->env_no_slot_keep ? 2 : 0), st);
    e->have_prev = true;
    for (int l = 0; l < use_free; ++l) {
      unsigned char* dl = e->dirty.as<unsigned char>() + (size_t)l * N;
      if (l > 0) td_launch_dirty_propagate(dl - N, src, N, K, dl, st);
      td_launch_rel_rows(dl, xm[cur], N, e->lig_rows.as<int>(), (int)e->lig_n_dst, e->row_pad, e->free_rows.as<int>() + (size_t)l * e->free_stride,
                         e->free_counts.as<int>() + 4 * l, st);
      e->launches += l > 0 ? 3 : 2;
    }
    td_launch_rel_compact(e->rel_flag.as<unsigned char>(), N, e->rel_list.as<int>(), e->n_rel.as<int>(), st);
    e->launches += 4;
    if (fused_logits(e) && e->restrict_last && last_blk && e->num_x2h > 0) {
      td_launch_rel_rows(e->rel_flag.as<unsigned char>(), xm[cur], N, e->lig_rows.as<int>(), (int)e->lig_n_dst, e->row_pad, e->rel_rows.as<int>(),
                         e->rel_counts.as<int>(), st);
      e->launches += 2;
    }
    const float4* xm_blk = xm[cur];
    const int NX = e->num_x2h, NH = e->num_h2x;
    const size_t L = e->layers.size();
    int g = 0;
    for (size_t l = 0; l < L && !(free_build && g >= free_build); ++l) {
      const TdLayer& ly = e->layers[l];
      const float* ew_x = e->ew_mode == 1 ? e->ew_x2h.as<float>() : e->e_w.as<float>();
      const float* ew_h = e->ew_mode == 1 ? e->ew_h2x.as<float>() : e->e_w.as<float>();
      const bool run_h2x = !free_build && !fix_x && Nl > 0 && NH > 0;
      const float* h_h2x = h;
      if (e->sync_twoup && run_h2x && NX > 0) {
        cudaMemcpyAsync(e->h_sync.p, h, (size_t)N * TD_H * 4, cudaMemcpyDeviceToDevice, st);
        h_h2x = e->h_sync.as<float>();
      }
      for (int i = 0; i < NX && !(free_build && g >= free_build); ++i, ++g) {
        const TdSubLayer& sx = ly.x2h[i];
        const int fl = g < use_free ? g : -1;
        node_side(e, h, N, sx, P, q, st);
        if (e->mlp_mode != 0 && (i == 0 || e->ew_mode == 1)) {
          TdEwR ew = {nullptr, nullptr, 0.f, 0.f, ly.offsets, ly.coeff, nullptr, nullptr};
          if (e->ew_mode == 1) {
            const TdSubLayer& sh0 = NH > 0 ? ly.h2x[0] : sx;
            ew.w_x2h = sx.ew_w; ew.w_h2x = sh0.ew_w; ew.b_x2h = sx.ew_b; ew.b_h2x = sh0.ew_b; ew.out_x2h = e->ew_x2h.as<float>(); ew.out_h2x = e->ew_h2x.as<float>();
          }
          td_launch_edge_geom(xm[cur], src, etype, N, K, e->dist.as<float>(), ew, st);
          e->launches += 1;
        }
        const bool fuse_agg = fused_logits(e) && K == 32 && !e->env_no_fused_agg && e->ew_mode != 2;
        const bool sub = fuse_agg && e->restrict_last && last_blk && l + 1 == L && i + 1 == NX && !e->env_no_restrict && !e->out_fc;
        const RowList rl = sub ? ROWS_RELEVANT : ROWS_ALL;
        float* agg_target = h;
        if (e->out_fc) {
          agg_target = e->hagg.as<float>();
          cudaMemsetAsync(agg_target, 0, (size_t)N * TD_H * 4, st);
        }
        {
          Prof pr(e, st, EV_EDGE_MLP);
          edge_mlp(e, P, xm[cur], src, etype, rl, K, sx.k, ly.offsets, ly.coeff, e->kbuf.as<float>(), st, ew_x, fused_logits(e) ? q : nullptr, nullptr,
                   nullptr, fuse_agg ? 1 : 0, fl);
          edge_mlp(e, P, xm[cur], src, etype, rl, K, sx.v, ly.offsets, ly.coeff, e->vbuf.as<float>(), st, ew_x, nullptr,
                   fuse_agg ? e->kbuf.as<float>() : nullptr, fuse_agg ? agg_target : nullptr, 0, fl);
        }
        if (!fuse_agg) {
          Prof pr(e, st, EV_AGG_H);
          if (fused_logits(e))
            td_launch_aggregate_h_logits(e->kbuf.as<float>(), e->vbuf.as<float>(), ew_x, src, e->out_fc ? agg_target : h, agg_target, N, K,
                                         e->ew_mode == 2 ? sx.ew_w : nullptr, sx.ew_b, st);
          else td_launch_aggregate_h(e->kbuf.as<float>(), e->vbuf.as<float>(), e->e_w.as<float>(), src, q, h, h, N, K, st);
        }
        e->launches += fuse_agg ? 4 : 5;
        if (e->out_fc) {
          float* t1 = P;
          float* t2 = P + (size_t)N * TD_H;
          TdMlp m1 = sx.out;
          m1.b2 = e->zeros128;
          td_launch_rows_tc(1, agg_target, TD_H, 0, N, m1, sx.out_wa_img, e->mlp_mode, t1, TD_H, 1, nullptr, nullptr, e->sm_count, st);
          m1.b2 = sx.out_b1;
          td_launch_rows_tc(1, h, TD_H, 0, N, m1, sx.out_wb_img, e->mlp_mode, t2, TD_H, 1, nullptr, nullptr, e->sm_count, st);
          td_launch_add_rows(t1, t2, t1, (long long)N * TD_H, st);
          td_launch_rows_tc(2, t1, TD_H, 0, N, sx.out, sx.out.w2_img, e->mlp_mode, t2, TD_H, 1, nullptr, nullptr, e->sm_count, st);
          td_launch_add_rows(h, t2, h, (long long)N * TD_H, st);
          e->launches += 6;
        }
        if (fl >= 0) {
          td_launch_restore_clean(e->dirty.as<unsigned char>() + (size_t)fl * N, xm_blk, e->h_free.as<float>() + (size_t)fl * N * TD_H, N, h, st);
          e->launches += 1;
        }
        if (free_build) cudaMemcpyAsync(e->h_free.as<float>() + (size_t)g * N * TD_H, h, (size_t)N * TD_H * 4, cudaMemcpyDeviceToDevice, st);
      }
      if (!run_h2x) continue;
      for (int j = 0; j < NH; ++j) {
        const TdSubLayer& sh = ly.h2x[j];
        if (j > 0 || NX == 0) {
          td_launch_edge_geom_rows(xm[cur], src, etype, e->lig_node.as<int>(), Nl, K, e->dist.as<float>(), e->ew_mode == 1 ? sh.ew_w : nullptr, sh.ew_b,
                                   ly.offsets, ly.coeff, e->ew_h2x.as<float>(), st);
          e->launches += 1;
        }
        {
          const bool rel = fused_logits(e) && !e->env_no_restrict;
          node_side(e, h_h2x, N, sh, P, q, st, rel ? e->rel_list.as<int>() : nullptr, rel ? e->n_rel.as<int>() : nullptr);
        }
        {
          Prof pr(e, st, EV_EDGE_MLP);
          edge_mlp(e, P, xm[cur], src, etype, ROWS_LIGAND, K, sh.k, ly.offsets, ly.coeff, e->kbuf.as<float>(), st, ew_h, fused_logits(e) ? q : nullptr);
          edge_mlp(e, P, xm[cur], src, etype, ROWS_LIGAND, K, sh.v, ly.offsets, ly.coeff, e->v16.as<float>(), st, ew_h);
        }
        {
          Prof pr(e, st, EV_AGG_X);
          if (fused_logits(e))
            td_launch_aggregate_x_logits(e->kbuf.as<float>(), e->v16.as<float>(), ew_h, src, xm[cur], e->lig_node.as<int>(), xm[cur ^ 1], Nl, K, st);
          else
            td_launch_aggregate_x(e->kbuf.as<float>(), e->v16.as<float>(), e->e_w.as<float>(), src, q, xm[cur], e->lig_node.as<int>(), xm[cur ^ 1], Nl, K, st);
        }
        e->launches += 5;
        cur ^= 1;
      }
    }
    if (Nl > 0) snapshot(blk + 1);
  }
  if (free_build) return;
  td_launch_head(h, e->lig_node.as<int>(), Nl, e->hd_w1t, e->hd_b1, e->hd_w2, e->hd_b2, e->cfg.num_classes, e->logits.as<float>(), st);
  e->launches += 1;
  e->final_buf = cur;
  e->have_graph = true;
  e->have_prev = true;
}
}

extern "C" int tdiff_set_time(tdiff_engine* e, const float* d_time_norm, void* stream) {
  if (!e || !e->bound) return set_err(TDIFF_ESTATE, "set_time before bind_batch");
  if (!e->time_emb) return TDIFF_OK;
  if (!d_time_norm) return set_err(TDIFF_EINVAL, "null time array");
  CK(cudaSetDevice(e->device));
  CK(cudaMemcpyAsync(e->time_norm.p, d_time_norm, (size_t)e->B * 4, cudaMemcpyDeviceToDevice, (cudaStream_t)stream));
  return TDIFF_OK;
}

namespace {
int forward_impl(tdiff_engine* e, float* d_pred_pos, float* d_pred_logits, float* d_final_h, int fix_x, float* d_block_pos, float* d_block_logits,
                 void* stream) {
  if (!e || !e->bound || !e->has_ligand) return set_err(TDIFF_ESTATE, "forward needs bind_batch + set_ligand first");
  cudaStream_t st = (cudaStream_t)stream;
  CK(cudaSetDevice(e->device));
  Prof* total = new Prof(e, st, EV_TOTAL);
  run_forward(e, st, fix_x, 0, d_block_pos, d_block_logits);
  delete total;
  const float4* xf = e->final_buf ? e->xm1.as<float4>() : e->xm0.as<float4>();
  if (d_pred_pos) { td_launch_gather_xyz(xf, e->lig_node.as<int>(), e->Nl, d_pred_pos, st); e->launches += 1; }
  if (d_pred_logits && e->Nl) CK(cudaMemcpyAsync(d_pred_logits, e->logits.p, (size_t)e->Nl * e->cfg.num_classes * 4, cudaMemcpyDeviceToDevice, st));
  if (d_final_h) CK(cudaMemcpyAsync(d_final_h, e->h.p, (size_t)e->N * TD_H * 4, cudaMemcpyDeviceToDevice, st));
  CK(cudaGetLastError());
  return TDIFF_OK;
}
}

extern "C" int tdiff_forward(tdiff_engine* e, float* d_pred_pos, float* d_pred_logits, float* d_final_h, int fix_x, void* stream) {
  return forward_impl(e, d_pred_pos, d_pred_logits, d_final_h, fix_x, nullptr, nullptr, stream);
}

extern "C" int tdiff_forward_blocks(tdiff_engine* e, float* d_pred_pos, float* d_pred_logits, float* d_final_h, int fix_x, float* d_block_pos,
                                    float* d_block_logits, void* stream) {
  return forward_impl(e, d_pred_pos, d_pred_logits, d_final_h, fix_x, d_block_pos, d_block_logits, stream);
}

extern "C" int64_t tdiff_num_edges(tdiff_engine* e, void* stream) {
  if (!e || !e->have_graph) return set_err(TDIFF_ESTATE, "no graph built yet (run forward first)");
  cudaStream_t st = (cudaStream_t)stream;
  if (cudaSetDevice(e->device) != cudaSuccess) return set_err(TDIFF_ECUDA, "cudaSetDevice failed");
  td_launch_edge_count_scan(e->src.as<int>(), e->N, e->K, e->node_off.as<long long>(), e->total_edges.as<long long>(), st);
  e->launches += 1;
  long long tot = 0;
  if (cudaMemcpyAsync(&tot, e->total_edges.p, 8, cudaMemcpyDeviceToHost, st) != cudaSuccess || cudaStreamSynchronize(st) != cudaSuccess)
    return set_err(TDIFF_ECUDA, "num_edges: %s", cudaGetErrorString(cudaGetLastError()));
  return tot;
}

extern "C" int tdiff_get_edge_index(tdiff_engine* e, int64_t* d_edge_index, void* stream) {
  if (!e || !e->have_graph || !d_edge_index) return set_err(TDIFF_ESTATE, "no graph built yet (run forward first)");
  cudaStream_t st = (cudaStream_t)stream;
  CK(cudaSetDevice(e->device));
  td_launch_edge_count_scan(e->src.as<int>(), e->N, e->K, e->node_off.as<long long>(), e->total_edges.as<long long>(), st);
  td_launch_edge_compact(e->src.as<int>(), nullptr, e->N, e->K, e->node_off.as<long long>(), e->total_edges.as<long long>(),
                         (long long*)d_edge_index, nullptr, st);
  e->launches += 2;
  CK(cudaGetLastError());
  return TDIFF_OK;
}

extern "C" int tdiff_get_edge_weight(tdiff_engine* e, float* d_e_w, void* stream) {
  if (!e || !e->have_graph || !d_e_w) return set_err(TDIFF_ESTATE, "no graph built yet (run forward first)");
  cudaStream_t st = (cudaStream_t)stream;
  CK(cudaSetDevice(e->device));
  td_launch_edge_count_scan(e->src.as<int>(), e->N, e->K, e->node_off.as<long long>(), e->total_edges.as<long long>(), st);
  td_launch_edge_compact(e->src.as<int>(), e->e_w.as<float>(), e->N, e->K, e->node_off.as<long long>(), e->total_edges.as<long long>(), nullptr,
                         d_e_w, st);
  e->launches += 2;
  CK(cudaGetLastError());
  return TDIFF_OK;
}

extern "C" int tdiff_get_node_pos(tdiff_engine* e, float* d_x, void* stream) {
  if (!e || !e->have_graph || !d_x) return set_err(TDIFF_ESTATE, "no forward run yet");
  CK(cudaSetDevice(e->device));
  td_launch_gather_xyz(e->final_buf ? e->xm1.as<float4>() : e->xm0.as<float4>(), nullptr, e->N, d_x, (cudaStream_t)stream);
  e->launches += 1;
  CK(cudaGetLastError());
  return TDIFF_OK;
}

namespace {
void build_free_cache(tdiff_engine* e, cudaStream_t st) {
  const size_t Nl = (size_t)e->Nl;
  char* sv = e->lig_save.as<char>();
  cudaMemcpyAsync(sv, e->lig_pos.p, Nl * 16, cudaMemcpyDeviceToDevice, st);
  cudaMemcpyAsync(sv + Nl * 16, e->lig_v.p, Nl * 4, cudaMemcpyDeviceToDevice, st);
  td_launch_park_ligand(e->lig_pos.as<float4>(), e->lig_v.as<int>(), e->Nl, st);
  const bool had_prev = e->have_prev;
  e->have_prev = false;
  run_forward(e, st, 1, e->free_depth);
  e->have_prev = false;
  (void)had_prev;
  cudaMemcpyAsync(e->lig_pos.p, sv, Nl * 16, cudaMemcpyDeviceToDevice, st);
  cudaMemcpyAsync(e->lig_v.p, sv + Nl * 16, Nl * 4, cudaMemcpyDeviceToDevice, st);
  e->launches += 1;
  e->free_ready = true;
}

void run_step(tdiff_engine* e, cudaStream_t st, const TdStepArgs& base) {
  if (e->time_emb) {
    td_launch_set_time(base.step, base.t_start, e->cfg.num_timesteps, e->B, e->time_norm.as<float>(), st);
    e->launches += 1;
  }
  e->restrict_last = true;
  run_forward(e, st, 0);
  e->restrict_last = false;
  TdStepArgs A = base;
  A.xm_final = e->final_buf ? e->xm1.as<float4>() : e->xm0.as<float4>();
  td_launch_step_epilogue(A, st);
  e->launches += 2;
}
}

extern "C" int tdiff_sample(tdiff_engine* e, int num_steps, const float* d_pos_noise, const float* d_v_uniform, uint64_t seed,
                            float* d_pos_traj, int64_t* d_v_traj, float* d_v0_traj, float* d_vt_traj, int pos_only, void* stream) {
  if (!e || !e->bound || !e->has_ligand) return set_err(TDIFF_ESTATE, "sample needs bind_batch + set_ligand first");
  const int T = e->cfg.num_timesteps;
  if (num_steps < 0 || num_steps > T) return set_err(TDIFF_EINVAL, "num_steps=%d outside 0..%d", num_steps, T);
  if ((d_pos_noise == nullptr) != (d_v_uniform == nullptr) && !pos_only)
    return set_err(TDIFF_EINVAL, "noise tape needs both pos_noise and v_uniform (or neither for Philox)");
  cudaStream_t st = (cudaStream_t)stream;
  CK(cudaSetDevice(e->device));
  if (num_steps == 0) return TDIFF_OK;
  TdStepArgs A;
  memset(&A, 0, sizeof(A));
  A.n_lig = e->Nl; A.n_classes = e->cfg.num_classes; A.t_start = T - 1; A.pos_only = pos_only;
  A.step = e->step.as<int>(); A.lig_node = e->lig_node.as<int>(); A.lig_graph = e->lig_graph.as<int>();
  A.logits = e->logits.as<float>(); A.offset = e->offset.as<float4>();
  A.c0 = e->t_c0; A.ct = e->t_ct; A.logvar = e->t_logvar; A.la_v = e->t_la; A.l1ma_v = e->t_l1ma; A.lca_v = e->t_lca; A.l1mca_v = e->t_l1mca;
  A.sra = e->t_sra; A.srm1 = e->t_srm1; A.mean_noise = e->cfg.model_mean_type == 1;
  A.log_k = (float)log((double)e->cfg.num_classes);
  A.pos_noise = d_pos_noise; A.v_uniform = d_v_uniform; A.seed = seed;
  A.lig_pos = e->lig_pos.as<float4>(); A.lig_v = e->lig_v.as<int>();
  A.pos_traj = d_pos_traj; A.v_traj = (long long*)d_v_traj; A.v0_traj = d_v0_traj; A.vt_traj = d_vt_traj;
  CK(cudaMemsetAsync(e->step.p, 0, sizeof(int), st));
  if (e->free_depth > 0 && !e->free_ready) build_free_cache(e, st);
  const bool eager = e->profiling || e->env_no_graph;
  Prof* total = new Prof(e, st, EV_TOTAL);
  run_step(e, st, A);
  int done = 1;
  if (!eager && num_steps > 2) {
    cudaStream_t cs = e->own_stream;
    CK(cudaEventRecord(e->ev_fork, st));
    CK(cudaStreamWaitEvent(cs, e->ev_fork, 0));
    cudaGraph_t graph = nullptr;
    cudaGraphExec_t exec = nullptr;
    const long long before = e->launches;
    cudaError_t ce = cudaStreamBeginCapture(cs, cudaStreamCaptureModeThreadLocal);
    if (ce == cudaSuccess) {
      run_step(e, cs, A);
      ce = cudaStreamEndCapture(cs, &graph);
    }
    const long long per_step = e->launches - before;
    e->launches = before;
    if (ce == cudaSuccess) ce = cudaGraphInstantiate(&exec, graph, 0);
    if (ce != cudaSuccess) {
      if (graph) cudaGraphDestroy(graph);
      (void)cudaGetLastError();
      delete total;
      return set_err(TDIFF_ECUDA, "CUDA graph capture of the sampling step failed: %s", cudaGetErrorString(ce));
    }
    for (; done < num_steps; ++done) {
      ce = cudaGraphLaunch(exec, cs);
      if (ce != cudaSuccess) break;
      e->launches += per_step;
    }
    if (ce == cudaSuccess) ce = cudaEventRecord(e->ev_join, cs);
    if (ce == cudaSuccess) ce = cudaStreamWaitEvent(st, e->ev_join, 0);
    cudaGraphExecDestroy(exec);
    cudaGraphDestroy(graph);
    if (ce != cudaSuccess) { delete total; return set_err(TDIFF_ECUDA, "cudaGraphLaunch failed: %s", cudaGetErrorString(ce)); }
  }
  for (; done < num_steps; ++done) run_step(e, st, A);
  delete total;
  CK(cudaGetLastError());
  return TDIFF_OK;
}

extern "C" int tdiff_sample_host(tdiff_engine* e, int B, const int32_t* pc, const int32_t* lc, const float* h_ppos, const float* h_pfeat,
                                 const float* h_lpos, const int64_t* h_lv, int center_mode, int num_steps, const float* h_pos_noise,
                                 const float* h_v_uniform, uint64_t seed, float* h_out_pos, int64_t* h_out_v, float* h_pos_traj,
                                 int64_t* h_v_traj, float* h_v0_traj, float* h_vt_traj, int pos_only, void* stream) {
  if (!e || !pc || !lc || B < 1) return set_err(TDIFF_EINVAL, "sample_host: bad arguments");
  cudaStream_t st = (cudaStream_t)stream;
  CK(cudaSetDevice(e->device));
  size_t Np = 0, Nl = 0;
  for (int g = 0; g < B; ++g) { Np += pc[g] > 0 ? pc[g] : 0; Nl += lc[g] > 0 ? lc[g] : 0; }
  const int F = e->cfg.protein_feat_dim, KC = e->cfg.num_classes;
  const size_t S = num_steps > 0 ? num_steps : 0;
  DevBuf* sb = e->stage;
  int bad = sb[0].ensure(Np * 12 + 16) | sb[1].ensure(Np * F * 4 + 16) | sb[2].ensure(Nl * 12 + 16) | sb[3].ensure(Nl * 8 + 16);
  if (h_pos_noise) bad |= sb[4].ensure(S * Nl * 12 + 16);
  if (h_v_uniform) bad |= sb[5].ensure(S * Nl * KC * 4 + 16);
  const size_t o_pos = 0, o_v = (o_pos + (h_pos_traj ? S * Nl * 12 : 0) + 15) / 16 * 16,
               o_v0 = (o_v + (h_v_traj ? S * Nl * 8 : 0) + 15) / 16 * 16,
               o_vt = o_v0 + (h_v0_traj ? S * Nl * KC * 4 : 0), o_end = o_vt + (h_vt_traj ? S * Nl * KC * 4 : 0);
  bad |= sb[6].ensure(o_end + 16) | sb[7].ensure(Nl * 12 + Nl * 8 + 32);
  if (bad) return set_err(TDIFF_ECUDA, "out of device memory staging host buffers");
  if (Np) {
    CK(cudaMemcpyAsync(sb[0].p, h_ppos, Np * 12, cudaMemcpyHostToDevice, st));
    CK(cudaMemcpyAsync(sb[1].p, h_pfeat, Np * F * 4, cudaMemcpyHostToDevice, st));
  }
  if (Nl) {
    CK(cudaMemcpyAsync(sb[2].p, h_lpos, Nl * 12, cudaMemcpyHostToDevice, st));
    CK(cudaMemcpyAsync(sb[3].p, h_lv, Nl * 8, cudaMemcpyHostToDevice, st));
  }
  if (h_pos_noise && S * Nl) CK(cudaMemcpyAsync(sb[4].p, h_pos_noise, S * Nl * 12, cudaMemcpyHostToDevice, st));
  if (h_v_uniform && S * Nl) CK(cudaMemcpyAsync(sb[5].p, h_v_uniform, S * Nl * KC * 4, cudaMemcpyHostToDevice, st));
  int rc = tdiff_bind_batch(e, B, pc, lc, sb[0].as<float>(), sb[1].as<float>(), center_mode, st);
  if (rc) return rc;
  rc = tdiff_set_ligand(e, sb[2].as<float>(), sb[3].as<int64_t>(), center_mode == 1, st);
  if (rc) return rc;
  char* tb = sb[6].as<char>();
  rc = tdiff_sample(e, num_steps, h_pos_noise ? sb[4].as<float>() : nullptr, h_v_uniform ? sb[5].as<float>() : nullptr, seed,
                    h_pos_traj ? (float*)(tb + o_pos) : nullptr, h_v_traj ? (int64_t*)(tb + o_v) : nullptr,
                    h_v0_traj ? (float*)(tb + o_v0) : nullptr, h_vt_traj ? (float*)(tb + o_vt) : nullptr, pos_only, st);
  if (rc) return rc;
  float* d_opos = sb[7].as<float>();
  int64_t* d_ov = (int64_t*)(sb[7].as<char>() + (Nl * 12 + 15) / 16 * 16);
  rc = tdiff_get_ligand(e, d_opos, d_ov, 1, st);
  if (rc) return rc;
  if (Nl) {
    if (h_out_pos) CK(cudaMemcpyAsync(h_out_pos, d_opos, Nl * 12, cudaMemcpyDeviceToHost, st));
    if (h_out_v) CK(cudaMemcpyAsync(h_out_v, d_ov, Nl * 8, cudaMemcpyDeviceToHost, st));
    if (S) {
      if (h_pos_traj) CK(cudaMemcpyAsync(h_pos_traj, tb + o_pos, S * Nl * 12, cudaMemcpyDeviceToHost, st));
      if (h_v_traj) CK(cudaMemcpyAsync(h_v_traj, tb + o_v, S * Nl * 8, cudaMemcpyDeviceToHost, st));
      if (h_v0_traj) CK(cudaMemcpyAsync(h_v0_traj, tb + o_v0, S * Nl * KC * 4, cudaMemcpyDeviceToHost, st));
      if (h_vt_traj) CK(cudaMemcpyAsync(h_vt_traj, tb + o_vt, S * Nl * KC * 4, cudaMemcpyDeviceToHost, st));
    }
  }
  CK(cudaStreamSynchronize(st));
  return TDIFF_OK;
}

extern "C" int tdiff_knn_graph(const float* d_x, int n_nodes, const int32_t* h_counts, int n_graphs, int k, int32_t* d_src_slots,
                               int64_t* d_edge_index, int64_t* h_n_edges, void* stream) {
  if (!d_x || !h_counts || !d_src_slots || n_nodes < 0 || n_graphs < 1 || k < 1 || k > TD_KMAX) return set_err(TDIFF_EINVAL, "knn_graph: bad arguments");
  cudaStream_t st = (cudaStream_t)stream;
  std::vector<int> ptr(n_graphs + 1, 0);
  int max_ng = 0;
  for (int g = 0; g < n_graphs; ++g) {
    if (h_counts[g] < 0) return set_err(TDIFF_EINVAL, "negative count");
    ptr[g + 1] = ptr[g] + h_counts[g];
    if (h_counts[g] > max_ng) max_ng = h_counts[g];
  }
  if (ptr[n_graphs] != n_nodes) return set_err(TDIFF_EINVAL, "graph counts sum to %d, expected %d nodes", ptr[n_graphs], n_nodes);
  if (max_ng > 2800) return set_err(TDIFF_EINVAL, "graph with %d nodes exceeds the k-NN kernel's shared-memory tile (2800)", max_ng);
  if (n_nodes == 0) { if (h_n_edges) *h_n_edges = 0; return TDIFF_OK; }
  DevBuf xm, dptr, off, tot;
  int rc = TDIFF_OK;
  if (xm.ensure((size_t)n_nodes * 16) || dptr.ensure((n_graphs + 1) * 4) || off.ensure((size_t)n_nodes * 8) || tot.ensure(8)) {
    rc = set_err(TDIFF_ECUDA, "out of device memory");
  } else {
    cudaMemcpyAsync(dptr.p, ptr.data(), (n_graphs + 1) * 4, cudaMemcpyHostToDevice, st);
    td_launch_pack_xyzm(d_x, nullptr, n_nodes, xm.as<float4>(), st);
    td_launch_knn(xm.as<float4>(), dptr.as<int>(), nullptr, n_graphs, max_ng, k, k, 0, d_src_slots, st);
    td_launch_edge_count_scan(d_src_slots, n_nodes, k, off.as<long long>(), tot.as<long long>(), st);
    if (d_edge_index) td_launch_edge_compact(d_src_slots, nullptr, n_nodes, k, off.as<long long>(), tot.as<long long>(), (long long*)d_edge_index, nullptr, st);
    long long t = 0;
    cudaMemcpyAsync(&t, tot.p, 8, cudaMemcpyDeviceToHost, st);
    cudaError_t ce = cudaStreamSynchronize(st);
    if (ce == cudaSuccess) ce = cudaGetLastError();
    if (ce != cudaSuccess) rc = set_err(TDIFF_ECUDA, "knn_graph: %s", cudaGetErrorString(ce));
    else if (h_n_edges) *h_n_edges = t;
  }
  xm.release(); dptr.release(); off.release(); tot.release();
  return rc;
}

extern "C" int tdiff_attn_aggregate_h(const float* d_k, const float* d_v, const float* d_e_w, const int32_t* d_src, const float* d_q,
                                      const float* d_h_in, float* d_h_out, int n_nodes, int kk, void* stream) {
  if (!d_k || !d_v || !d_e_w || !d_src || !d_q || !d_h_in || !d_h_out || n_nodes < 0 || kk < 1 || kk > TD_KMAX)
    return set_err(TDIFF_EINVAL, "attn_aggregate_h: bad arguments");
  td_launch_aggregate_h(d_k, d_v, d_e_w, d_src, d_q, d_h_in, d_h_out, n_nodes, kk, (cudaStream_t)stream);
  CK(cudaGetLastError());
  return TDIFF_OK;
}

extern "C" int tdiff_attn_aggregate_x(const float* d_k, const float* d_v16, const float* d_e_w, const int32_t* d_src, const float* d_q,
                                      const float* d_x, const uint8_t* d_mask, float* d_x_out, int n_nodes, int kk, void* stream) {
  if (!d_k || !d_v16 || !d_e_w || !d_src || !d_q || !d_x || !d_mask || !d_x_out || n_nodes < 0 || kk < 1 || kk > TD_KMAX)
    return set_err(TDIFF_EINVAL, "attn_aggregate_x: bad arguments");
  cudaStream_t st = (cudaStream_t)stream;
  if (n_nodes == 0) return TDIFF_OK;
  DevBuf a, b;
  if (a.ensure((size_t)n_nodes * 16) || b.ensure((size_t)n_nodes * 16)) { a.release(); b.release(); return set_err(TDIFF_ECUDA, "out of device memory"); }
  td_launch_pack_xyzm(d_x, d_mask, n_nodes, a.as<float4>(), st);
  td_launch_aggregate_x(d_k, d_v16, d_e_w, d_src, d_q, a.as<float4>(), nullptr, b.as<float4>(), n_nodes, kk, st);
  td_launch_gather_xyz(b.as<float4>(), nullptr, n_nodes, d_x_out, st);
  cudaError_t ce = cudaStreamSynchronize(st);
  if (ce == cudaSuccess) ce = cudaGetLastError();
  a.release(); b.release();
  if (ce != cudaSuccess) return set_err(TDIFF_ECUDA, "attn_aggregate_x: %s", cudaGetErrorString(ce));
  return TDIFF_OK;
}

extern "C" int tdiff_scatter_mean3(const float* d_src, const int32_t* h_counts, int n_segments, float* d_out, void* stream) {
  if (!d_src || !h_counts || !d_out || n_segments < 1) return set_err(TDIFF_EINVAL, "scatter_mean3: bad arguments");
  cudaStream_t st = (cudaStream_t)stream;
  std::vector<int> ptr(n_segments + 1, 0);
  for (int g = 0; g < n_segments; ++g) ptr[g + 1] = ptr[g] + (h_counts[g] > 0 ? h_counts[g] : 0);
  DevBuf dptr, o4;
  if (dptr.ensure((n_segments + 1) * 4) || o4.ensure((size_t)n_segments * 16)) { dptr.release(); o4.release(); return set_err(TDIFF_ECUDA, "out of device memory"); }
  cudaMemcpyAsync(dptr.p, ptr.data(), (n_segments + 1) * 4, cudaMemcpyHostToDevice, st);
  td_launch_segment_mean3(d_src, dptr.as<int>(), n_segments, o4.as<float4>(), st);
  td_launch_gather_xyz(o4.as<float4>(), nullptr, n_segments, d_out, st);
  cudaError_t ce = cudaStreamSynchronize(st);
  if (ce == cudaSuccess) ce = cudaGetLastError();
  dptr.release(); o4.release();
  if (ce != cudaSuccess) return set_err(TDIFF_ECUDA, "scatter_mean3: %s", cudaGetErrorString(ce));
  return TDIFF_OK;
}

extern "C" int tdiff_check_stability(const float* d_pos, const int32_t* d_atomic_num, const int32_t* h_counts, int n_mol, int hs, int32_t* d_nr_bonds,
                                     int32_t* d_stable_atoms, uint8_t* d_mol_stable, void* stream) {
  if (!d_pos || !d_atomic_num || !h_counts || !d_stable_atoms || !d_mol_stable || n_mol < 0) return set_err(TDIFF_EINVAL, "check_stability: bad arguments");
  if (n_mol == 0) return TDIFF_OK;
  cudaStream_t st = (cudaStream_t)stream;
  std::vector<int> ptr(n_mol + 1, 0);
  for (int m = 0; m < n_mol; ++m) {
    if (h_counts[m] < 0) return set_err(TDIFF_EINVAL, "negative atom count");
    ptr[m + 1] = ptr[m] + h_counts[m];
  }
  DevBuf dptr, derr;
  if (dptr.ensure((n_mol + 1) * 4) || derr.ensure(4)) { dptr.release(); derr.release(); return set_err(TDIFF_ECUDA, "out of device memory"); }
  cudaMemcpyAsync(dptr.p, ptr.data(), (n_mol + 1) * 4, cudaMemcpyHostToDevice, st);
  cudaMemsetAsync(derr.p, 0, 4, st);
  td_launch_check_stability(d_pos, d_atomic_num, dptr.as<int>(), n_mol, hs, d_nr_bonds, d_stable_atoms, d_mol_stable, derr.as<int>(), st);
  int flag = 0;
  cudaMemcpyAsync(&flag, derr.p, 4, cudaMemcpyDeviceToHost, st);
  cudaError_t ce = cudaStreamSynchronize(st);
  if (ce == cudaSuccess) ce = cudaGetLastError();
  dptr.release(); derr.release();
  if (ce != cudaSuccess) return set_err(TDIFF_ECUDA, "check_stability: %s", cudaGetErrorString(ce));
  if (flag) return set_err(TDIFF_EINVAL, "check_stability: atomic number outside the reference's table (H C N O F P S Cl)");
  return TDIFF_OK;
}

extern "C" int64_t tdiff_launch_count(tdiff_engine* e) { return e ? e->launches : 0; }
extern "C" int tdiff_edge_mlp_mode(tdiff_engine* e) { return !e ? TDIFF_EINVAL : (e->mlp_mode == 2 && e->mlp_v4) ? 5 : e->mlp_mode; }

extern "C" int tdiff_profile(tdiff_engine* e, int enable) {
  if (!e) return set_err(TDIFF_EINVAL, "null engine");
  e->profiling = enable != 0;
  if (enable) {
    for (int i = 0; i < EV_KINDS; ++i) { e->ms_acc[i] = 0; e->n_acc[i] = 0; }
  }
  return TDIFF_OK;
}

extern "C" int tdiff_profile_read(tdiff_engine* e, double* ms_h, int64_t* n_h, double* ms_x, int64_t* n_x, double* ms_mlp, int64_t* n_mlp,
                                  double* ms_total) {
  if (!e) return set_err(TDIFF_EINVAL, "null engine");
  CK(cudaSetDevice(e->device));
  CK(cudaDeviceSynchronize());
  for (auto& ev : e->events) {
    float ms = 0.f;
    if (cudaEventElapsedTime(&ms, ev.a, ev.b) == cudaSuccess) { e->ms_acc[ev.kind] += ms; e->n_acc[ev.kind] += 1; }
    cudaEventDestroy(ev.a); cudaEventDestroy(ev.b);
  }
  e->events.clear();
  if (ms_h) *ms_h = e->ms_acc[EV_AGG_H];
  if (n_h) *n_h = e->n_acc[EV_AGG_H];
  if (ms_x) *ms_x = e->ms_acc[EV_AGG_X];
  if (n_x) *n_x = e->n_acc[EV_AGG_X];
  if (ms_mlp) *ms_mlp = e->ms_acc[EV_EDGE_MLP];
  if (n_mlp) *n_mlp = e->n_acc[EV_EDGE_MLP];
  if (ms_total) *ms_total = e->ms_acc[EV_TOTAL];
  return TDIFF_OK;
}
```

### targetdiff_b200/csrc/hopper_mma.cuh

```cuda
#pragma once
#include <stdint.h>

__device__ __forceinline__ uint64_t gmma_desc_sw128(uint32_t smem_addr) {
  return (uint64_t)((smem_addr >> 4) & 0x3FFF) | ((uint64_t)1 << 16) | ((uint64_t)(1024 >> 4) << 32) | ((uint64_t)1 << 62);
}
__device__ __forceinline__ void wgmma_fence() { asm volatile("wgmma.fence.sync.aligned;" ::: "memory"); }
__device__ __forceinline__ void wgmma_commit() { asm volatile("wgmma.commit_group.sync.aligned;" ::: "memory"); }
__device__ __forceinline__ void wgmma_wait_all() { asm volatile("wgmma.wait_group.sync.aligned 0;" ::: "memory"); }

__device__ __forceinline__ void wgmma_n128(float (&d)[64], uint64_t desc_a, uint64_t desc_b, uint32_t accumulate) {
  asm volatile(
      "{\n\t.reg .pred p;\n\tsetp.ne.b32 p, %66, 0;\n\t"
      "wgmma.mma_async.sync.aligned.m64n128k16.f32.bf16.bf16 {%0,%1,%2,%3,%4,%5,%6,%7,%8,%9,%10,%11,%12,%13,%14,%15,%16,%17,%18,%19,%20,%21,%22,%23,%24,%25,%26,%27,%28,%29,%30,%31,%32,%33,%34,%35,%36,%37,%38,%39,%40,%41,%42,%43,%44,%45,%46,%47,%48,%49,%50,%51,%52,%53,%54,%55,%56,%57,%58,%59,%60,%61,%62,%63}, %64, %65, p, 1, 1, 0, 0;\n\t}"
      : "+f"(d[0]), "+f"(d[1]), "+f"(d[2]), "+f"(d[3]), "+f"(d[4]), "+f"(d[5]), "+f"(d[6]), "+f"(d[7]), "+f"(d[8]), "+f"(d[9]), "+f"(d[10]), "+f"(d[11]), "+f"(d[12]), "+f"(d[13]), "+f"(d[14]), "+f"(d[15]), "+f"(d[16]), "+f"(d[17]), "+f"(d[18]), "+f"(d[19]), "+f"(d[20]), "+f"(d[21]), "+f"(d[22]), "+f"(d[23]), "+f"(d[24]), "+f"(d[25]), "+f"(d[26]), "+f"(d[27]), "+f"(d[28]), "+f"(d[29]), "+f"(d[30]), "+f"(d[31]), "+f"(d[32]), "+f"(d[33]), "+f"(d[34]), "+f"(d[35]), "+f"(d[36]), "+f"(d[37]), "+f"(d[38]), "+f"(d[39]), "+f"(d[40]), "+f"(d[41]), "+f"(d[42]), "+f"(d[43]), "+f"(d[44]), "+f"(d[45]), "+f"(d[46]), "+f"(d[47]), "+f"(d[48]), "+f"(d[49]), "+f"(d[50]), "+f"(d[51]), "+f"(d[52]), "+f"(d[53]), "+f"(d[54]), "+f"(d[55]), "+f"(d[56]), "+f"(d[57]), "+f"(d[58]), "+f"(d[59]), "+f"(d[60]), "+f"(d[61]), "+f"(d[62]), "+f"(d[63])
      : "l"(desc_a), "l"(desc_b), "r"(accumulate) : "memory");
}

__device__ __forceinline__ void wgmma_n128_rs(float (&d)[64], const uint32_t (&a)[4], uint64_t desc_b, uint32_t accumulate) {
  asm volatile(
      "{\n\t.reg .pred p;\n\tsetp.ne.b32 p, %69, 0;\n\t"
      "wgmma.mma_async.sync.aligned.m64n128k16.f32.bf16.bf16 {%0,%1,%2,%3,%4,%5,%6,%7,%8,%9,%10,%11,%12,%13,%14,%15,%16,%17,%18,%19,%20,%21,%22,%23,%24,%25,%26,%27,%28,%29,%30,%31,%32,%33,%34,%35,%36,%37,%38,%39,%40,%41,%42,%43,%44,%45,%46,%47,%48,%49,%50,%51,%52,%53,%54,%55,%56,%57,%58,%59,%60,%61,%62,%63}, {%64,%65,%66,%67}, %68, p, 1, 1, 0;\n\t}"
      : "+f"(d[0]), "+f"(d[1]), "+f"(d[2]), "+f"(d[3]), "+f"(d[4]), "+f"(d[5]), "+f"(d[6]), "+f"(d[7]), "+f"(d[8]), "+f"(d[9]), "+f"(d[10]), "+f"(d[11]), "+f"(d[12]), "+f"(d[13]), "+f"(d[14]), "+f"(d[15]), "+f"(d[16]), "+f"(d[17]), "+f"(d[18]), "+f"(d[19]), "+f"(d[20]), "+f"(d[21]), "+f"(d[22]), "+f"(d[23]), "+f"(d[24]), "+f"(d[25]), "+f"(d[26]), "+f"(d[27]), "+f"(d[28]), "+f"(d[29]), "+f"(d[30]), "+f"(d[31]), "+f"(d[32]), "+f"(d[33]), "+f"(d[34]), "+f"(d[35]), "+f"(d[36]), "+f"(d[37]), "+f"(d[38]), "+f"(d[39]), "+f"(d[40]), "+f"(d[41]), "+f"(d[42]), "+f"(d[43]), "+f"(d[44]), "+f"(d[45]), "+f"(d[46]), "+f"(d[47]), "+f"(d[48]), "+f"(d[49]), "+f"(d[50]), "+f"(d[51]), "+f"(d[52]), "+f"(d[53]), "+f"(d[54]), "+f"(d[55]), "+f"(d[56]), "+f"(d[57]), "+f"(d[58]), "+f"(d[59]), "+f"(d[60]), "+f"(d[61]), "+f"(d[62]), "+f"(d[63])
      : "r"(a[0]), "r"(a[1]), "r"(a[2]), "r"(a[3]), "l"(desc_b), "r"(accumulate) : "memory");
}

__device__ __forceinline__ void wgmma_n32_rs(float (&d)[16], const uint32_t (&a)[4], uint64_t desc_b, uint32_t accumulate) {
  asm volatile(
      "{\n\t.reg .pred p;\n\tsetp.ne.b32 p, %21, 0;\n\t"
      "wgmma.mma_async.sync.aligned.m64n32k16.f32.bf16.bf16 {%0,%1,%2,%3,%4,%5,%6,%7,%8,%9,%10,%11,%12,%13,%14,%15}, {%16,%17,%18,%19}, %20, p, 1, 1, 0;\n\t}"
      : "+f"(d[0]), "+f"(d[1]), "+f"(d[2]), "+f"(d[3]), "+f"(d[4]), "+f"(d[5]), "+f"(d[6]), "+f"(d[7]), "+f"(d[8]), "+f"(d[9]), "+f"(d[10]), "+f"(d[11]),
        "+f"(d[12]), "+f"(d[13]), "+f"(d[14]), "+f"(d[15])
      : "r"(a[0]), "r"(a[1]), "r"(a[2]), "r"(a[3]), "l"(desc_b), "r"(accumulate) : "memory");
}

__device__ __forceinline__ void wgmma_n16_rs(float (&d)[8], const uint32_t (&a)[4], uint64_t desc_b, uint32_t accumulate) {
  asm volatile(
      "{\n\t.reg .pred p;\n\tsetp.ne.b32 p, %13, 0;\n\t"
      "wgmma.mma_async.sync.aligned.m64n16k16.f32.bf16.bf16 {%0,%1,%2,%3,%4,%5,%6,%7}, {%8,%9,%10,%11}, %12, p, 1, 1, 0;\n\t}"
      : "+f"(d[0]), "+f"(d[1]), "+f"(d[2]), "+f"(d[3]), "+f"(d[4]), "+f"(d[5]), "+f"(d[6]), "+f"(d[7])
      : "r"(a[0]), "r"(a[1]), "r"(a[2]), "r"(a[3]), "l"(desc_b), "r"(accumulate) : "memory");
}
```

### targetdiff_b200/csrc/tdiff_common.cuh

```cuda
#pragma once
#include <cuda_runtime.h>
#include <stdint.h>

#define TD_H 128
#define TD_HEADS 16
#define TD_HD 8
#define TD_NG 20
#define TD_TAB 21
#define TD_KMAX 64
#define TD_NPROJ 640
#define TD_CMAX 24

struct TdMlp {
  const float* tab;
  const float* ln_g;
  const float* ln_b;
  const float* w2t;
  const float* b2;
  int nout;
  int offA, offB;
  const unsigned char* w2_img;
  const unsigned char* tabcls_img;
};

struct TdEwR {
  const float* w_x2h;
  const float* w_h2x;
  float b_x2h, b_h2x;
  const float* offsets;
  float coeff;
  float* out_x2h;
  float* out_h2x;
};

struct TdSubLayer {
  const float* wn_t;
  const float* bn;
  const unsigned char* wn_img;
  TdMlp k, v, q;
  const float* ew_w;
  float ew_b;
  const unsigned char* out_wa_img;
  const unsigned char* out_wb_img;
  const float* out_b1;
  TdMlp out;
};

__device__ __forceinline__ float warp_sum(float v) {
#pragma unroll
  for (int o = 16; o > 0; o >>= 1) v += __shfl_xor_sync(0xffffffffu, v, o);
  return v;
}
__device__ __forceinline__ float warp_max(float v) {
#pragma unroll
  for (int o = 16; o > 0; o >>= 1) v = fmaxf(v, __shfl_xor_sync(0xffffffffu, v, o));
  return v;
}

__device__ __forceinline__ void ln_relu_128(float (&p)[4], const float* __restrict__ g, const float* __restrict__ b, int lane) {
  float s = warp_sum((p[0] + p[1]) + (p[2] + p[3]));
  float mean = s * (1.0f / 128.0f);
  float d0 = p[0] - mean, d1 = p[1] - mean, d2 = p[2] - mean, d3 = p[3] - mean;
  float var = warp_sum((d0 * d0 + d1 * d1) + (d2 * d2 + d3 * d3)) * (1.0f / 128.0f);
  float rstd = 1.0f / sqrtf(var + 1e-5f);
  p[0] = fmaxf(d0 * rstd * g[lane] + b[lane], 0.0f);
  p[1] = fmaxf(d1 * rstd * g[lane + 32] + b[lane + 32], 0.0f);
  p[2] = fmaxf(d2 * rstd * g[lane + 64] + b[lane + 64], 0.0f);
  p[3] = fmaxf(d3 * rstd * g[lane + 96] + b[lane + 96], 0.0f);
}

#define TD_LDA 132
#define TD_GEMM_THREADS 512

__device__ __forceinline__ void tile_gemm_128(const float* __restrict__ As, const float* __restrict__ Bs, float (&acc)[4][8],
                                              int ty, int tx) {
#pragma unroll
  for (int i = 0; i < 4; ++i)
#pragma unroll
    for (int j = 0; j < 8; ++j) acc[i][j] = 0.0f;
#pragma unroll 2
  for (int kk = 0; kk < 128; kk += 4) {
    float4 a[4];
#pragma unroll
    for (int i = 0; i < 4; ++i) a[i] = *reinterpret_cast<const float4*>(As + (ty + 32 * i) * TD_LDA + kk);
#pragma unroll
    for (int k4 = 0; k4 < 4; ++k4) {
      float4 b0 = *reinterpret_cast<const float4*>(Bs + (kk + k4) * 128 + 4 * tx);
      float4 b1 = *reinterpret_cast<const float4*>(Bs + (kk + k4) * 128 + 64 + 4 * tx);
#pragma unroll
      for (int i = 0; i < 4; ++i) {
        float av = (k4 == 0) ? a[i].x : (k4 == 1) ? a[i].y : (k4 == 2) ? a[i].z : a[i].w;
        acc[i][0] = fmaf(av, b0.x, acc[i][0]);
        acc[i][1] = fmaf(av, b0.y, acc[i][1]);
        acc[i][2] = fmaf(av, b0.z, acc[i][2]);
        acc[i][3] = fmaf(av, b0.w, acc[i][3]);
        acc[i][4] = fmaf(av, b1.x, acc[i][4]);
        acc[i][5] = fmaf(av, b1.y, acc[i][5]);
        acc[i][6] = fmaf(av, b1.z, acc[i][6]);
        acc[i][7] = fmaf(av, b1.w, acc[i][7]);
      }
    }
  }
}

#define TD_MAX_DEVICES 64
template <class Kernel>
inline void td_opt_in_smem(Kernel kernel, size_t bytes, size_t (&done)[TD_MAX_DEVICES]) {
  int dev = 0;
  const bool known = cudaGetDevice(&dev) == cudaSuccess && dev >= 0 && dev < TD_MAX_DEVICES;
  if (known && bytes <= done[dev]) return;
  cudaFuncSetAttribute(kernel, cudaFuncAttributeMaxDynamicSharedMemorySize, (int)bytes);
  if (known) done[dev] = bytes;
}

void td_launch_knn(const float4* xm, const int* node_ptr, const int* prot_ptr, int n_graphs, int max_nodes_per_graph, int k, int stride, int hybrid,
                   int* src, cudaStream_t st);
void td_launch_knn_cache(const float4* xm, const int* node_ptr, const int* prot_ptr, int n_graphs, int max_ng, int k, unsigned long long* cache,
                         cudaStream_t st);
void td_launch_knn_update(const float4* xm, const int* node_ptr, const int* prot_ptr, int n_graphs, int max_ng, int k, int stride, int hybrid,
                          const unsigned long long* cache, int* src, cudaStream_t st);
void td_launch_edge_const(const float4* xm, const int* src, int* src_prev, int have_prev, int n_nodes, int k, const float* offsets, float coeff,
                          const float* w1t, const float* b1, const float* ln_g, const float* ln_b, const float* w2, float b2,
                          unsigned char* etype, float* e_w, unsigned char* rel_flag, unsigned char* touch_flag, int* work_list, int* n_work,
                          int gate_mode, cudaStream_t st);
void td_launch_dirty_propagate(const unsigned char* in, const int* src, int n_nodes, int k, unsigned char* out, cudaStream_t st);
void td_launch_restore_clean(const unsigned char* dirty, const float4* xm, const float* h_free, int n_nodes, float* h, cudaStream_t st);
void td_launch_rel_rows(const unsigned char* rel_flag, const float4* xm, int n_nodes, const int* lig_rows, int n_lig_rows, int pad, int* rel_rows,
                        int* rel_counts, cudaStream_t st);
void td_launch_protein_embed(const float* feat, int n_protein, int fdim, const float* w, const float* b, const int* prot_node,
                             float* h0, cudaStream_t st);
void td_launch_init_h(const float* h0, const float4* xm, const int* lig_v, const int* node_lig, const float* wl_t, const float* bl,
                      const float* w_time, const float* time_norm, const int* lig_graph, int n_nodes, float* h, cudaStream_t st);
void td_launch_node_proj(const float* h, int n_nodes, const float* wn_t, const float* bn, float* P, cudaStream_t st);
void td_launch_node_q(const float* P, int n_nodes, TdMlp q, float* qout, cudaStream_t st);
void td_launch_edge_mlp(const float* P, const float4* xm, const int* src, const unsigned char* etype, const int* row_nodes,
                        long long n_rows, int k, TdMlp m, const float* offsets, float coeff, float* out, int sm_count, cudaStream_t st);
void td_launch_edge_geom(const float4* xm, const int* src, const unsigned char* etype, int n_nodes, int k, float* dist, const TdEwR& ew, cudaStream_t st);
void td_launch_edge_geom_rows(const float4* xm, const int* src, const unsigned char* etype, const int* rows, int n_rows, int k, float* dist,
                              const float* gate_w, float gate_b, const float* offsets, float coeff, float* gate, cudaStream_t st);
void td_launch_add_rows(const float* a, const float* b, float* out, long long n_floats, cudaStream_t st);
void td_launch_set_time(const int* step, int t_start, int n_timesteps, int n_graphs, float* time_norm, cudaStream_t st);
void td_launch_edge_mlp_tc(const float* P, const float4* xm, const int* src, const unsigned char* etype, const float* dist,
                           const int* row_nodes, long long n_rows, int k, TdMlp m, const unsigned char* w2_image, int pieces, const float* offsets, float coeff,
                           float* out, int sm_count, cudaStream_t st);
void td_launch_edge_mlp_v4(const float* P, int zero_row, const int* src, const unsigned char* etype, const float* dist, const int* row_nodes, long long n_dst,
                           long long split_dst, const int* d_counts, int k, const TdMlp& m, const float* h_offsets, float coeff,
                           const float* h_ln_b, const float* h_b2, const float* qnode, float* out, int out_by_slot,
                           const float* agg_logits, const float* agg_e_w, float* agg_h, int key_softmax, int sm_count, cudaStream_t st);
void td_launch_rows_tc(int mode, const float* in, int ldi, int in_off, long long n_rows, TdMlp m, const unsigned char* w_image, int pieces, float* out,
                       int ldo, int nblocks, const int* row_list, const int* d_n_rows, int sm_count, cudaStream_t st);
void td_launch_rel_compact(const unsigned char* flag, int n_nodes, int* rel_list, int* n_rel, cudaStream_t st);
void td_launch_aggregate_h(const float* kbuf, const float* vbuf, const float* e_w, const int* src, const float* q, const float* h_in,
                           float* h_out, int n_nodes, int k, cudaStream_t st);
void td_launch_aggregate_x(const float* kbuf, const float* v16, const float* e_w, const int* src, const float* q, const float4* xm_in,
                           const int* row_nodes, float4* xm_out, int n_rows, int k, cudaStream_t st);
void td_launch_aggregate_h_logits(const float* logits, const float* vbuf, const float* e_w, const int* src, const float* h_in, float* h_out,
                                  int n_nodes, int k, const float* ewm_w, float ewm_b, cudaStream_t st);
void td_launch_aggregate_x_logits(const float* logits, const float* v16, const float* e_w, const int* src, const float4* xm_in,
                                  const int* row_nodes, float4* xm_out, int n_rows, int k, cudaStream_t st);
void td_launch_head(const float* h, const int* lig_node, int n_lig, const float* w1t, const float* b1, const float* w2, const float* b2,
                    int n_classes, float* logits, cudaStream_t st);
void td_launch_check_stability(const float* pos, const int* atomic_num, const int* mol_ptr, int n_mol, int hs, int* nr_bonds, int* stable_atoms,
                               unsigned char* mol_stable, int* err, cudaStream_t st);
```

Baseline: 17.57.

## Fold attention-weighted aggregation before the value MLP's second GEMM

Adds an AGG variant of the edge MLP kernel for the value MLP with k=32. It first reduces the post-LayerNorm hidden activations over neighbours, weighted by the attention logits and using mma.sync. Only after that does it apply the per-head W2 slice, so the full 128x128 second GEMM per edge is no longer computed. The bias is added using the summed weights. The cost is a new per-head W2 layout, extra staging of logits and h through TMA, a single ordering phase, and a path that only applies to specific shapes. It can be turned off with an env var.

```diff
diff --git a/targetdiff_b200/csrc/edge_mlp_v4.cu b/targetdiff_b200/csrc/edge_mlp_v4.cu
--- a/targetdiff_b200/csrc/edge_mlp_v4.cu
+++ b/targetdiff_b200/csrc/edge_mlp_v4.cu
@@ -15,12 +15,14 @@
 constexpr int kSrcStride = 512 + 32, kDst = 8;
 constexpr int sSrc = 0, sDstRows = sSrc + kTile * kSrcStride, sMeta = sDstRows + kDst * 512, kStage = sMeta + kTile * 16;
 constexpr int kMAtom = 32 * 128, kMPiece = 2 * kMAtom, kMImg = 2 * kMPiece;
-template <bool FOLD>
+constexpr int kAggX = 17 * 32 * 8, kWgtRows = kTile * 64;
+template <bool FOLD, bool AGG = false>
 struct Map {
-  static constexpr int W = 0, T = W + 4 * 128 * 128, Par = T + (FOLD ? 1 : 2) * kTabClassBytes, X = Par + 2 * 128 * 4,
-                       M = X + kCons * 4 * 2 * 128 * 4, C = M + (FOLD ? kCons * kMImg : 0), Stage = C + (FOLD ? kCons * 32 * 4 : 0),
-                       Bar = Stage + kCons * kStage, Smem = Bar + 8 * (1 + 2 * kCons);
-  static_assert(M % 1024 == 0 && Stage % 128 == 0 && kStage % 128 == 0 && Smem <= 227 * 1024, "shared-memory map");
+  static constexpr int W = 0, T = W + 4 * 128 * 128, Par = T + (FOLD || AGG ? 1 : 2) * kTabClassBytes, X = Par + 2 * 128 * 4,
+                       M = X + kCons * 4 * (AGG ? kAggX : 2 * 128 * 4), C = M + (FOLD ? kCons * kMImg : 0),
+                       Stage = C + (FOLD ? kCons * 32 * 4 : 0), StageBytes = kStage + (AGG ? kWgtRows : 0),
+                       Bar = Stage + kCons * StageBytes, Smem = Bar + 8 * (1 + 2 * kCons);
+  static_assert(M % 1024 == 0 && Stage % 128 == 0 && StageBytes % 128 == 0 && Smem <= 227 * 1024, "shared-memory map");
 };
 constexpr int kOrderBar = 5;
 constexpr int kFoldBar = 7;
@@ -94,7 +96,7 @@
 
 using namespace v4;
 
-template <int NOUT, bool FOLD>
+template <int NOUT, bool FOLD, bool AGG = false>
 __global__ void __launch_bounds__(kThreads, 1)
 edge_mlp_v4_kernel(const float* __restrict__ P, int zero_row, const int* __restrict__ src, const unsigned char* __restrict__ etype,
                    const float* __restrict__ dist_arr, const int* __restrict__ row_nodes, long long n_dst, long long split_dst,
@@ -102,7 +104,8 @@
                    const unsigned char* __restrict__ tab_image, float coeff, const float* __restrict__ qnode, float* __restrict__ out, int out_by_slot, AggArgs agg,
                    int fold_cls, const __grid_constant__ LnParams lp) {
   static_assert(!FOLD || NOUT == 128, "the fold applies to the key MLPs");
-  using L = Map<FOLD>;
+  static_assert(!AGG || (NOUT == 128 && !FOLD), "the aggregation fold applies to the value MLPs");
+  using L = Map<FOLD, AGG>;
   extern __shared__ __align__(1024) unsigned char smem_raw[];
   const uint32_t sbase = smem_u32(smem_raw);
   const uint32_t sW = sbase + L::W, sT = sbase + L::T, sBar = sbase + L::Bar;
@@ -121,7 +124,7 @@
   if (d_counts) { n_dst = d_counts[0]; split_dst = d_counts[1]; }
   const long long n_rows = n_dst * k, split_rows = split_dst * k;
   long long row_lo = 0, row_hi = n_rows;
-  if constexpr (FOLD) { if (fold_cls) row_lo = split_rows; else row_hi = split_rows; }
+  if constexpr (FOLD || AGG) { if (fold_cls) row_lo = split_rows; else row_hi = split_rows; }
   const long long n_tiles = row_hi > row_lo ? (row_hi - row_lo + kTile - 1) / kTile : 0;
   const long long my_tiles = (n_tiles > blockIdx.x) ? (n_tiles - blockIdx.x + gridDim.x - 1) / gridDim.x : 0;
   auto full_bar = [&](int c) { return sBar + 8u * (1 + c); };
@@ -133,7 +136,7 @@
     mbar_init(sBar, 1);
     for (int c = 0; c < kCons; ++c) { mbar_init(full_bar(c), 32); mbar_init(empty_bar(c), 128); }
     fence_barrier_init();
-    if constexpr (FOLD) {
+    if constexpr (FOLD || AGG) {
       mbar_expect_tx(sBar, 4u * 128 * 128 + kTabClassBytes);
       bulk_g2s(sW, w2_image, 4u * 128 * 128, sBar);
       bulk_g2s(sT, tab_image + (size_t)fold_cls * kTabClassBytes, kTabClassBytes, sBar);
@@ -150,7 +153,7 @@
     setmaxnreg_dec<kProdRegs>();
     if (warp >= kCons) return;
     const int c = warp;
-    const uint32_t st = sbase + L::Stage + (uint32_t)c * kStage;
+    const uint32_t st = sbase + L::Stage + (uint32_t)c * L::StageBytes;
     for (long long it = c, use = 0; it < my_tiles; it += kCons, ++use) {
       const long long tile = blockIdx.x + it * (long long)gridDim.x, row0 = row_lo + tile * kTile;
       int j0;
@@ -180,14 +183,16 @@
       if (lane < n_d) dnode = row_nodes[a0 + lane];
       mbar_wait(empty_bar(c), (uint32_t)(use & 1) ^ 1u);
 #pragma unroll
-      for (int h = 0; h < 2; ++h) *reinterpret_cast<int4*>(smem_raw + L::Stage + c * kStage + sMeta + 16 * (lane + 32 * h)) = meta[h];
-      if (lane == 0) mbar_expect_tx_only(full_bar(c), (uint32_t)(kTile + (FOLD ? 2 : 1) * n_d) * 512u);
+      for (int h = 0; h < 2; ++h) *reinterpret_cast<int4*>(smem_raw + L::Stage + c * L::StageBytes + sMeta + 16 * (lane + 32 * h)) = meta[h];
+      if (lane == 0) mbar_expect_tx_only(full_bar(c), (uint32_t)(kTile + (FOLD || AGG ? 2 : 1) * n_d) * 512u + (AGG ? kWgtRows : 0u));
       __syncwarp();
 #pragma unroll
       for (int h = 0; h < 2; ++h)
         bulk_g2s(st + sSrc + (uint32_t)(lane + 32 * h) * kSrcStride, P + (size_t)(s[h] >= 0 ? s[h] : zero_row) * TD_NPROJ + offB, 512u, full_bar(c));
       if (lane < n_d) bulk_g2s(st + sDstRows + (uint32_t)lane * 512u, P + (size_t)(dnode >= 0 ? dnode : zero_row) * TD_NPROJ + offA, 512u, full_bar(c));
       if (FOLD && lane < n_d) bulk_g2s(st + sDstRows + (uint32_t)(2 + lane) * 512u, qnode + (size_t)(dnode >= 0 ? dnode : 0) * TD_H, 512u, full_bar(c));
+      if (AGG && lane < n_d) bulk_g2s(st + sDstRows + (uint32_t)(2 + lane) * 512u, agg.h + (size_t)(dnode >= 0 ? dnode : 0) * TD_H, 512u, full_bar(c));
+      if (AGG && lane == 0) bulk_g2s(st + kStage, agg.logits + (size_t)row0 * TD_HEADS, kWgtRows, full_bar(c));
       mbar_arrive(full_bar(c));
     }
     return;
@@ -207,13 +212,14 @@
   float* const xpart = xslot + ((w & 1) ? -256 : 256);
   const bool do_agg = !FOLD && NOUT == 128 && qnode == nullptr && agg.logits != nullptr;
   const bool key_sm = NOUT == 128 && qnode != nullptr && agg.key_softmax;
-  const unsigned char* const stage = smem_raw + L::Stage + cwg * kStage;
+  const unsigned char* const stage = smem_raw + L::Stage + cwg * L::StageBytes;
   const int ct = tid & 127, fu = ct & 7, fg = ct >> 3;
   const int fhd = 8 * (fg & 1) + 4 * (fu >> 2) + (fu & 3), fs = fu >> 2, frun = (fg >> 1) ^ (((fu >> 1) & 1) << 2);
   const int fn0 = 16 * ((fhd >> 1) & 1) + 2 * (fhd >> 2) + (fhd & 1);
   unsigned char* const mimg = smem_raw + L::M + cwg * kMImg;
   float* const s_c = reinterpret_cast<float*>(smem_raw + L::C) + cwg * 32;
   const int srow = k == 32 ? (w >> 1) : 0;
+  constexpr int kPhases = AGG ? 1 : 2;
   const int order_mine = kOrderBar + cwg, order_other = kOrderBar + (cwg ^ 1);
   const long long n_iter = (my_tiles + kCons - 1) / kCons;
   if (n_iter == 0) return;
@@ -223,11 +229,11 @@
   for (long long n = 0; n < n_iter; ++n, set ^= 1) {
     const long long it = n * kCons + cwg;
     if (it >= my_tiles) {
-      for (int phase = 0; phase < 2; ++phase) { named_bar_sync(order_mine, 256); named_bar_arrive(order_other, 256); }
+      for (int phase = 0; phase < kPhases; ++phase) { named_bar_sync(order_mine, 256); named_bar_arrive(order_other, 256); }
       continue;
     }
     const long long tile = blockIdx.x + it * (long long)gridDim.x, row0 = row_lo + tile * kTile;
-    const int cls = FOLD ? 0 : (row0 >= split_rows) ? 1 : 0;
+    const int cls = (FOLD || AGG) ? 0 : (row0 >= split_rows) ? 1 : 0;
     long long idx[2];
     int node[2], s[2], ty[2], jj[2], dsl[2];
     float dist[2];
@@ -256,6 +262,17 @@
           }
           qf[sl][hf] = v;
         }
+    }
+    float wf[8], hst[2];
+    const int ccol = 64 * (w & 1) + 2 * lane;
+    if constexpr (AGG) {
+      const float* const ws = reinterpret_cast<const float*>(stage + kStage) + (16 * w + 2 * q) * TD_HEADS + (lane >> 2);
+#pragma unroll
+      for (int r = 0; r < 4; ++r)
+#pragma unroll
+        for (int c = 0; c < 2; ++c) wf[2 * r + c] = ws[(8 * (r >> 1) + c) * TD_HEADS + 8 * (r & 1)];
+      const float2 hv = *reinterpret_cast<const float2*>(stage + sDstRows + (2 + (w >> 1)) * 512 + 4 * ccol);
+      hst[0] = hv.x; hst[1] = hv.y;
     }
     uint32_t ghi[4][4], glo[4][4];
 #pragma unroll
@@ -377,6 +394,60 @@
         const float y0 = __fmaf_rn(x[e], rstd[h], b.x), y1 = __fmaf_rn(x[e + 1], rstd[h], b.y);
         split2(fmaxf(y0, 0.f), fmaxf(y1, 0.f), ahi[kk][r], alo[kk][r]);
       }
+    if constexpr (AGG) {
+      uint32_t whi[4], wlo[4];
+#pragma unroll
+      for (int r = 0; r < 4; ++r) split2(wf[2 * r], wf[2 * r + 1], whi[r], wlo[r]);
+      float u[17][4];
+#pragma unroll
+      for (int j = 0; j < 16; ++j) {
+        const int kk = j >> 1, r0 = 2 * (j & 1);
+        const uint32_t bh0 = movmatrix_trans(ahi[kk][r0]), bh1 = movmatrix_trans(ahi[kk][r0 + 1]);
+        const uint32_t bl0 = movmatrix_trans(alo[kk][r0]), bl1 = movmatrix_trans(alo[kk][r0 + 1]);
+        u[j][0] = u[j][1] = u[j][2] = u[j][3] = 0.f;
+        mma_m16n8k16(u[j], whi, bh0, bh1);
+        mma_m16n8k16(u[j], whi, bl0, bl1);
+        mma_m16n8k16(u[j], wlo, bh0, bh1);
+      }
+      constexpr uint32_t kOnes = 0x3f803f80u;
+      u[16][0] = u[16][1] = u[16][2] = u[16][3] = 0.f;
+      mma_m16n8k16(u[16], whi, kOnes, kOnes);
+      mma_m16n8k16(u[16], wlo, kOnes, kOnes);
+      float2* const xmine = reinterpret_cast<float2*>(smem_raw + L::X + (cwg * 4 + w) * kAggX) + lane;
+      const float2* const xpeer = reinterpret_cast<const float2*>(smem_raw + L::X + (cwg * 4 + (w ^ 1)) * kAggX) + lane;
+      const bool odd = w & 1;
+#pragma unroll
+      for (int j = 0; j < 17; ++j) xmine[32 * j] = odd ? make_float2(u[j][0], u[j][1]) : make_float2(u[j][2], u[j][3]);
+      named_bar_sync(pair_bar, 64);
+      float uu[17][2];
+#pragma unroll
+      for (int j = 0; j < 17; ++j) {
+        const float2 v = xpeer[32 * j];
+        uu[j][0] = (odd ? u[j][2] : u[j][0]) + v.x;
+        uu[j][1] = (odd ? u[j][3] : u[j][1]) + v.y;
+      }
+      named_bar_sync(pair_bar, 64);
+      const int hd = (lane >> 2) + 8 * (w & 1), xo = 16 * (hd & 1);
+      const float* const w2a = reinterpret_cast<const float*>(smem_raw + L::W) + hd * 1024 + 4 * q + xo;
+      const float* const w2b = reinterpret_cast<const float*>(smem_raw + L::W) + hd * 1024 + 4 * q + 16 - xo;
+      float p[8];
+#pragma unroll
+      for (int d = 0; d < 8; ++d) p[d] = 0.f;
+#pragma unroll
+      for (int j = 0; j < 16; ++j)
+#pragma unroll
+        for (int t = 0; t < 4; ++t) {
+          const float4 c4 = *reinterpret_cast<const float4*>(((t & 1) ? w2b : w2a) + 64 * j + 32 * (t >> 1));
+          p[2 * t] = __fmaf_rn(c4.y, uu[j][1], __fmaf_rn(c4.x, uu[j][0], p[2 * t]));
+          p[2 * t + 1] = __fmaf_rn(c4.w, uu[j][1], __fmaf_rn(c4.z, uu[j][0], p[2 * t + 1]));
+        }
+      transpose_reduce<8, 2, 0>(p, lane);
+      if (node[0] >= 0) {
+        const float2 bb = *reinterpret_cast<const float2*>(s_b2 + ccol);
+        stg64(agg.h + (size_t)node[0] * TD_H + ccol, hst[0] + __fmaf_rn(bb.x, uu[16][0], p[0]), hst[1] + __fmaf_rn(bb.y, uu[16][0], p[1]));
+      }
+      continue;
+    }
     float o[NOUT / 2];
     if constexpr (FOLD) {
       named_bar_sync(kFoldBar + cwg, 128);
@@ -430,7 +501,6 @@
       const long long dslot = tile * 2 + (w >> 1);
       const int dnode = dslot < n_dst ? row_nodes[dslot] : -1;
       const bool active = dnode >= 0;
-      const int ccol = 64 * (w & 1) + 2 * lane;
       float2 hin = make_float2(0.f, 0.f);
       if (active) hin = *reinterpret_cast<const float2*>(agg.h + (size_t)dnode * TD_H + ccol);
       float wt[2][16];
@@ -557,17 +627,19 @@
 void td_launch_edge_mlp_v4(const float* P, int zero_row, const int* src, const unsigned char* etype, const float* dist, const int* row_nodes, long long n_dst,
                            long long split_dst, const int* d_counts, int k, const TdMlp& m, const float* h_offsets, float coeff,
                            const float* h_ln_b, const float* h_b2, const float* qnode, float* out, int out_by_slot,
-                           const float* agg_logits, const float* agg_e_w, float* agg_h, int key_softmax, int sm_count, cudaStream_t st) {
+                           const float* agg_logits, const float* agg_e_w, float* agg_h, int key_softmax, int agg_fold, int sm_count,
+                           cudaStream_t st) {
   if (n_dst == 0) return;
   LnParams lp;
   memcpy(lp.b, h_ln_b, sizeof(lp.b));
   memset(lp.b2, 0, sizeof(lp.b2));
   memcpy(lp.b2, h_b2, sizeof(float) * (size_t)m.nout);
   memcpy(lp.mu, h_offsets, sizeof(lp.mu));
-  static size_t opted128[TD_MAX_DEVICES] = {0}, opted16[TD_MAX_DEVICES] = {0}, optedF[TD_MAX_DEVICES] = {0};
+  static size_t opted128[TD_MAX_DEVICES] = {0}, opted16[TD_MAX_DEVICES] = {0}, optedF[TD_MAX_DEVICES] = {0}, optedA[TD_MAX_DEVICES] = {0};
   td_opt_in_smem(edge_mlp_v4_kernel<128, false>, Map<false>::Smem, opted128);
   td_opt_in_smem(edge_mlp_v4_kernel<16, false>, Map<false>::Smem, opted16);
   td_opt_in_smem(edge_mlp_v4_kernel<128, true>, Map<true>::Smem, optedF);
+  td_opt_in_smem(edge_mlp_v4_kernel<128, false, true>, Map<false, true>::Smem, optedA);
   auto grid_of = [&](long long n_dst_range) {
     const long long n_tiles = (n_dst_range * k + kTile - 1) / kTile;
     return (int)(n_tiles < sm_count ? n_tiles : sm_count);
@@ -584,6 +656,13 @@
         edge_mlp_v4_kernel<128, true><<<grid_of(n_cls[cls]), kThreads, Map<true>::Smem, st>>>(
             P, zero_row, src, etype, dist, row_nodes, n_dst, split_dst, d_counts, k, m.offA, m.offB,
             reinterpret_cast<const unsigned char*>(m.w2t), m.tabcls_img, coeff, qnode, out, out_by_slot, agg, cls, lp);
+  } else if (agg_fold && k == 32 && !qnode && agg_logits && m.w2h) {
+    const long long n_cls[2] = {split_dst, n_dst - split_dst};
+    for (int cls = 0; cls < 2; ++cls)
+      if (n_cls[cls] > 0)
+        edge_mlp_v4_kernel<128, false, true><<<grid_of(n_cls[cls]), kThreads, Map<false, true>::Smem, st>>>(
+            P, zero_row, src, etype, dist, row_nodes, n_dst, split_dst, d_counts, k, m.offA, m.offB,
+            reinterpret_cast<const unsigned char*>(m.w2h), m.tabcls_img, coeff, nullptr, out, out_by_slot, agg, cls, lp);
   } else {
     edge_mlp_v4_kernel<128, false><<<grid_of(n_dst), kThreads, Map<false>::Smem, st>>>(
         P, zero_row, src, etype, dist, row_nodes, n_dst, split_dst, d_counts, k, m.offA, m.offB, m.w2_img, m.tabcls_img, coeff, qnode, out,
diff --git a/targetdiff_b200/csrc/engine.cu b/targetdiff_b200/csrc/engine.cu
--- a/targetdiff_b200/csrc/engine.cu
+++ b/targetdiff_b200/csrc/engine.cu
@@ -79,7 +79,7 @@
   bool restrict_last = false;
   bool knn_incremental = false;
   bool have_prev = false;
-  bool env_no_fused_agg = false, env_no_restrict = false, env_no_graph = false, env_knn_full = false, env_no_slot_keep = false;
+  bool env_no_fused_agg = false, env_no_agg_fold = false, env_no_restrict = false, env_no_graph = false, env_knn_full = false, env_no_slot_keep = false;
   int B = 0, N = 0, Np = 0, Nl = 0, K = 0, max_ng = 0, final_buf = 0;
   int KQ = 0, hybrid = 0;
   DevBuf node_ptr, prot_ptr, prot_node, prot_graph, lig_node, lig_graph, node_lig;
@@ -126,7 +126,7 @@
   }
 };
 
-struct MlpOff { size_t tab, ln_g, ln_b, w2t, b2; int nout; long long img, tabcls; };
+struct MlpOff { size_t tab, ln_g, ln_b, w2t, b2; int nout; long long img, tabcls, w2h = -1; };
 
 inline uint16_t bf16_rn(float x) {
   uint32_t u; memcpy(&u, &x, 4);
@@ -230,6 +230,18 @@
   return true;
 }
 
+void pack_w2_heads(Packer& pk, MlpOff& o) {
+  o.w2h = (long long)pk.alloc((size_t)TD_H * TD_H);
+  float* img = &pk.host[(size_t)o.w2h];
+  const float* w2t = &pk.host[o.w2t];
+  for (int hd = 0; hd < TD_HEADS; ++hd)
+    for (int d = 0; d < 8; ++d)
+      for (int f = 0; f < TD_H; ++f) {
+        const int j = f / 8, q = (f % 8) / 2, c = f % 2, t = d / 2;
+        img[hd * 1024 + j * 64 + ((t ^ (hd & 1)) * 4 + q) * 4 + 2 * (d % 2) + c] = w2t[(size_t)f * TD_H + 8 * hd + d];
+      }
+}
+
 struct SubOff {
   size_t wn_t, bn; long long wn_img; MlpOff k, v, q;
   long long ew_w = -1; float ew_b = 0.f;
@@ -279,6 +291,7 @@
   const float *w1k = nullptr, *w1v = nullptr;
   if (!pack_edge_mlp(pk, p + "." + kn, TD_H, sign_in_w1, so.k, &w1k)) return false;
   if (!pack_edge_mlp(pk, p + "." + vn, nout_v, sign_in_w1, so.v, &w1v)) return false;
+  if (nout_v == TD_H) pack_w2_heads(pk, so.v);
   const std::string qp = p + "." + qn;
   const float* w1q = pk.get(qp + ".net.0.weight", (int64_t)TD_H * TD_H);
   const float* b1q = pk.get(qp + ".net.0.bias", TD_H);
@@ -326,6 +339,7 @@
   m.w2_img = (o.img >= 0 && img_base) ? img_base + o.img : nullptr;
   m.tabcls_img = (o.tabcls >= 0 && img_base) ? img_base + o.tabcls : nullptr;
   m.tab = base + o.tab; m.ln_g = base + o.ln_g; m.ln_b = base + o.ln_b; m.w2t = base + o.w2t; m.b2 = base + o.b2;
+  m.w2h = o.w2h >= 0 ? base + o.w2h : nullptr;
   m.nout = o.nout; m.offA = offA; m.offB = offB;
   return m;
 }
@@ -489,6 +503,7 @@
     return set_err(TDIFF_EINVAL, "num_x2h / num_h2x != 1 and sync_twoup are implemented (and tested) in the default engine mode only (unset TDIFF_EDGE_MLP)");
   }
   e->env_no_fused_agg = getenv("TDIFF_NO_FUSED_AGG") != nullptr;
+  e->env_no_agg_fold = getenv("TDIFF_NO_AGG_FOLD") != nullptr;
   e->env_no_restrict = getenv("TDIFF_NO_RESTRICT") != nullptr;
   e->env_no_graph = getenv("TDIFF_NO_GRAPH") != nullptr;
   e->env_knn_full = getenv("TDIFF_KNN_FULL") != nullptr;
@@ -744,7 +759,7 @@
     td_launch_edge_mlp_v4(P, e->N, src, etype, e->dist.as<float>(), rows, n_dst, split, counts, K, m,
                           e->host_arena.data() + (offsets - e->arena), coeff, e->host_arena.data() + (m.ln_b - e->arena),
                           e->host_arena.data() + (m.b2 - e->arena), qnode, out, by_slot, agg_logits, e_w, agg_h, key_softmax,
-                          e->sm_count, st);
+                          e->env_no_agg_fold ? 0 : 1, e->sm_count, st);
     return;
   }
   const int* row_nodes = list == ROWS_LIGAND ? e->lig_node.as<int>() : nullptr;
diff --git a/targetdiff_b200/csrc/hopper_mma.cuh b/targetdiff_b200/csrc/hopper_mma.cuh
--- a/targetdiff_b200/csrc/hopper_mma.cuh
+++ b/targetdiff_b200/csrc/hopper_mma.cuh
@@ -40,3 +40,14 @@
       : "+f"(d[0]), "+f"(d[1]), "+f"(d[2]), "+f"(d[3]), "+f"(d[4]), "+f"(d[5]), "+f"(d[6]), "+f"(d[7])
       : "r"(a[0]), "r"(a[1]), "r"(a[2]), "r"(a[3]), "l"(desc_b), "r"(accumulate) : "memory");
 }
+
+__device__ __forceinline__ void mma_m16n8k16(float (&d)[4], const uint32_t (&a)[4], uint32_t b0, uint32_t b1) {
+  asm volatile("mma.sync.aligned.m16n8k16.row.col.f32.bf16.bf16.f32 {%0,%1,%2,%3}, {%4,%5,%6,%7}, {%8,%9}, {%0,%1,%2,%3};"
+               : "+f"(d[0]), "+f"(d[1]), "+f"(d[2]), "+f"(d[3])
+               : "r"(a[0]), "r"(a[1]), "r"(a[2]), "r"(a[3]), "r"(b0), "r"(b1));
+}
+__device__ __forceinline__ uint32_t movmatrix_trans(uint32_t a) {
+  uint32_t d;
+  asm volatile("movmatrix.sync.aligned.m8n8.trans.b16 %0, %1;" : "=r"(d) : "r"(a));
+  return d;
+}
diff --git a/targetdiff_b200/csrc/tdiff_common.cuh b/targetdiff_b200/csrc/tdiff_common.cuh
--- a/targetdiff_b200/csrc/tdiff_common.cuh
+++ b/targetdiff_b200/csrc/tdiff_common.cuh
@@ -21,6 +21,7 @@
   int offA, offB;
   const unsigned char* w2_img;
   const unsigned char* tabcls_img;
+  const float* w2h;
 };
 
 struct TdEwR {
@@ -146,7 +147,8 @@
 void td_launch_edge_mlp_v4(const float* P, int zero_row, const int* src, const unsigned char* etype, const float* dist, const int* row_nodes, long long n_dst,
                            long long split_dst, const int* d_counts, int k, const TdMlp& m, const float* h_offsets, float coeff,
                            const float* h_ln_b, const float* h_b2, const float* qnode, float* out, int out_by_slot,
-                           const float* agg_logits, const float* agg_e_w, float* agg_h, int key_softmax, int sm_count, cudaStream_t st);
+                           const float* agg_logits, const float* agg_e_w, float* agg_h, int key_softmax, int agg_fold, int sm_count,
+                           cudaStream_t st);
 void td_launch_rows_tc(int mode, const float* in, int ldi, int in_off, long long n_rows, TdMlp m, const unsigned char* w_image, int pieces, float* out,
                        int ldo, int nblocks, const int* row_list, const int* d_n_rows, int sm_count, cudaStream_t st);
 void td_launch_rel_compact(const unsigned char* flag, int n_nodes, int* rel_list, int* n_rel, cudaStream_t st);
```

New measurement: 17.78 (median of 6 runs). 1.01x the previous value.
